# jacobkrantz/VLN-CE

Measured on AMD Instinct MI355X. Metric: policy-steps/sec (fwd+bwd), higher is better.
Workload: dtype f32

## Files before the change

### include/vlnce_hip.h

```cpp
#ifndef VLNCE_HIP_H
#define VLNCE_HIP_H

#include <stddef.h>
#include <stdint.h>

#ifdef __cplusplus
extern "C" {
#endif

typedef void* vlnce_stream_t;

enum { VLNCE_ACT_NONE = 0, VLNCE_ACT_RELU = 1, VLNCE_ACT_SIGMOID = 2, VLNCE_ACT_TANH = 3 };

int vlnce_version(void);
int vlnce_option_count(void);
int vlnce_option_index(const char* name);
const char* vlnce_last_error(void);

int vlnce_set_option(const char* name, int value);
int vlnce_get_option(const char* name, int* value);
int vlnce_option_default(const char* name, int* value);

typedef struct {
  int N, H, W, Cin;
  int Cout, KH, KW;
  int stride, pad;
  int Ho, Wo;
  int ldx, ldy;
} vlnce_conv_desc;

typedef struct {
  const float* x;
  int Cin, ldx;
  const void* w_frag;
  const float* in_scale;
  const float* in_shift;
  const float* in_center;
  int in_relu;
} vlnce_regen;

typedef struct {
  const float* in_scale;
  const float* in_shift;
  const float* in_center;
  int in_relu;
  const float* x2;
  const float* in2_scale;
  const float* in2_shift;
  const float* in2_center;
  float* side_out;
  const void* w_split;
  const void* w_frag;
  const int* options;
  int w_format;
  const vlnce_regen* regen;
} vlnce_prologue;

#define VLNCE_BN_SHARDS 16
typedef struct {
  double* acc;
  void* workspace;
  long workspace_bytes;
} vlnce_bn_sums;

typedef struct {
  const float* scale;
  const float* shift;
  const float* residual;
  int ldr;
  int act;
  int accumulate;
  float* stat_partial;
  const vlnce_bn_sums* bn;
  int stats_only;
} vlnce_epilogue;

long vlnce_conv2d_bn_workspace_bytes(const vlnce_conv_desc* d);
int vlnce_bn_finalize_sums(double* acc, int M, int C, const float* gamma, const float* beta,
                           float eps, float momentum, float* running_mean, float* running_var,
                           float* scale_out, float* shift_out, float* mean_out, float* rstd_out,
                           vlnce_stream_t stream);

int vlnce_conv2d_tiles_m(const vlnce_conv_desc* d);
int vlnce_conv2d_tile_rows(const vlnce_conv_desc* d);

int vlnce_conv2d_split_weights(const float* w, void* planes, long count, int format,
                               vlnce_stream_t stream);

long vlnce_conv2d_pack_bytes(const vlnce_conv_desc* d);
int vlnce_conv2d_pack_weights(const float* w_ohwi, void* frag, const vlnce_conv_desc* d,
                              int format , vlnce_stream_t stream);

typedef struct vlnce_weight_job {
  const float* w_oihw;
  void* dst;
  int Cout, Cin, T;
  int kind;
  int transposed;
  int format;
} vlnce_weight_job;
long vlnce_weight_job_items(const vlnce_weight_job* job);
int vlnce_conv2d_prepare_weights(const vlnce_weight_job* jobs_dev, const long* first_item_dev,
                                 int njobs, long total_items, vlnce_stream_t stream);

#define VLNCE_CONV_PATH_F32 0
#define VLNCE_CONV_PATH_X3 1
#define VLNCE_CONV_PATH_P3 2
#define VLNCE_CONV_PATH_M3 3
int vlnce_conv2d_last_path(void);

#define VLNCE_CONV_KERNEL(family, format, kernel, a, b, c) \
  ((family) | ((format) << 2) | ((kernel) << 4) | ((a) << 8) | ((b) << 16) | ((c) << 24))
#define VLNCE_CONV_KERNEL_FAMILY(v) ((v) & 3)
#define VLNCE_CONV_KERNEL_FORMAT(v) (((v) >> 2) & 3)
#define VLNCE_CONV_KERNEL_KIND(v) (((v) >> 4) & 15)
#define VLNCE_CONV_KERNEL_A(v) (((v) >> 8) & 255)
#define VLNCE_CONV_KERNEL_B(v) (((v) >> 16) & 255)
#define VLNCE_CONV_KERNEL_C(v) (((v) >> 24) & 127)
#define VLNCE_CONV_KERNEL_P3 0
#define VLNCE_CONV_KERNEL_U3 1
#define VLNCE_CONV_KERNEL_S3 2
#define VLNCE_CONV_KERNEL_R3 3
#define VLNCE_CONV_P3_DENSE 0
#define VLNCE_CONV_P3_GATHER 1
#define VLNCE_CONV_P3_DUAL 2
#define VLNCE_CONV_KERNEL_F32_BUF 0
#define VLNCE_CONV_KERNEL_F32_SPLITK 1
#define VLNCE_CONV_KERNEL_F32_V4 2
#define VLNCE_CONV_KERNEL_F32_S 3
#define VLNCE_CONV_KERNEL_F32_STEM3 4
#define VLNCE_CONV_KERNEL_F32_STEM1 5
#define VLNCE_CONV_KERNEL_F32_DUAL 6
int vlnce_conv2d_last_kernel(void);

int vlnce_conv2d_fwd(const float* x, const float* w_ohwi, float* y,
                     const vlnce_conv_desc* d, const vlnce_prologue* pro,
                     const vlnce_epilogue* epi, vlnce_stream_t stream);

int vlnce_gemm(const float* A, int lda, int transA, const float* B, int ldb, int transB,
               float* C, int ldc, int M, int N, int K,
               const vlnce_epilogue* epi, vlnce_stream_t stream);

#define VLNCE_GEMM_KERNEL(a, b, tile, splitk, zero, pass2) \
  ((a) | ((b) << 2) | ((tile) << 4) | ((zero) ? 1 << 6 : 0) | ((pass2) ? 1 << 7 : 0) | ((splitk) << 8))
#define VLNCE_GEMM_KERNEL_A(v) ((v) & 3)
#define VLNCE_GEMM_KERNEL_B(v) (((v) >> 2) & 3)
#define VLNCE_GEMM_KERNEL_TILE(v) (((v) >> 4) & 3)
#define VLNCE_GEMM_KERNEL_ZERO(v) (((v) >> 6) & 1)
#define VLNCE_GEMM_KERNEL_PASS2(v) (((v) >> 7) & 1)
#define VLNCE_GEMM_KERNEL_SPLITK(v) (((v) >> 8) & 255)
#define VLNCE_GEMM_A_BUF 0
#define VLNCE_GEMM_A_IM2COL_V4 1
#define VLNCE_GEMM_A_IM2COL_S 2
#define VLNCE_GEMM_A_TRANS 3
#define VLNCE_GEMM_B_BUF 0
#define VLNCE_GEMM_B_NK_V4 1
#define VLNCE_GEMM_B_NK_S 2
#define VLNCE_GEMM_B_KN 3
#define VLNCE_GEMM_TILE_128X128 1
#define VLNCE_GEMM_TILE_128X64 2
#define VLNCE_GEMM_TILE_64X64 3
int vlnce_gemm_last_kernel(void);

int vlnce_linear_rows_supported(int M, int N, int K);
int vlnce_linear_rows_fwd(const float* x, int ldx, const float* w, int ldw, const float* bias,
                          int act, float* y, int ldy, int M, int N, int K, vlnce_stream_t stream);
int vlnce_linear_rows_bwd(const float* x, int ldx, const float* w, int ldw, const float* dy,
                          int lddy, const float* y, int ldy, int act, float* dx, float* dw,
                          float* db, int M, int N, int K, vlnce_stream_t stream);

int vlnce_colsum(const float* x, int ldx, int M, int N, float* out, int accumulate,
                 vlnce_stream_t stream);

size_t vlnce_bn_finalize_workspace_bytes(int tiles_m, int C);
int vlnce_bn_finalize(const float* stat_partial, int tiles_m, int tile_rows, int M, int C,
                      const float* gamma, const float* beta, float eps, float momentum,
                      float* running_mean, float* running_var,
                      float* scale_out, float* shift_out,
                      float* mean_out, float* rstd_out,
                      void* workspace, size_t workspace_bytes,
                      vlnce_stream_t stream);

int vlnce_scale_shift_act(const float* x, const float* scale, const float* shift,
                          const float* center, int rows_per_sample, const float* residual,
                          float* y, long M, int C, int act, vlnce_stream_t stream);

int vlnce_scale_shift_add_act(const float* x1, const float* scale1, const float* shift1,
                              const float* center1, const float* x2, const float* scale2,
                              const float* shift2, const float* center2, float* y, long M, int C,
                              int act, vlnce_stream_t stream);

int vlnce_gn_chunks(int HW);
int vlnce_gn_partial(const float* x, int Nimg, int HW, int C, float* partial ,
                     vlnce_stream_t stream);
int vlnce_gn_finalize(const float* partial, int Nimg, int HW, int C, int groups,
                      const float* gamma, const float* beta, float eps,
                      float* scale_out, float* shift_out,
                      float* center_out,
                      float* mean_out, float* rstd_out,
                      vlnce_stream_t stream);
int vlnce_gn_finalize_tiles(const float* stat_partial, int tile_rows, int Nimg, int HW, int C,
                            int groups, const float* gamma, const float* beta, float eps,
                            float* scale_out, float* shift_out, float* center_out,
                            float* mean_out, float* rstd_out, vlnce_stream_t stream);
int vlnce_group_norm_small(const float* x, int Nimg, int HW, int C, int groups, const float* gamma,
                           const float* beta, float eps, const float* residual, int act, float* y,
                           vlnce_stream_t stream);

int vlnce_maxpool3x3s2(const float* x, float* y, int N, int H, int W, int C, int Ho, int Wo,
                       const float* in_scale, const float* in_shift, const float* in_center,
                       int in_relu, vlnce_stream_t stream);
int vlnce_avgpool2x2(const float* x, float* y, int N, int H, int W, int C, vlnce_stream_t stream);

int vlnce_space_to_depth2(const float* x, float* y, int N, int H, int W, int C, int pad_lo,
                          int pad_hi, const float* scale, const float* shift,
                          vlnce_stream_t stream);
#define VLNCE_DT_F32 0
#define VLNCE_DT_U8 1
typedef struct {
  const void* x;
  const void* x2;
  const unsigned char* mask2;
  int dtype;
  int N, F, Hs, Ws, C;
  int y0, x0, H, W;
} vlnce_frames;
int vlnce_frames_s2d(const vlnce_frames* frames, float* y, int pad_lo, int pad_hi,
                     const float* scale, const float* shift, vlnce_stream_t stream);
int vlnce_stem7_fwd(const vlnce_frames* frames, const float* in_scale, const float* in_shift,
                    const void* w_frag, int w_format, float* y, int Cout, const vlnce_epilogue* epi,
                    vlnce_stream_t stream);
int vlnce_frames_avgpool2(const vlnce_frames* frames, float* y, vlnce_stream_t stream);
int vlnce_frames_f32(const vlnce_frames* frames, float* y, const float* scale, const float* shift,
                     vlnce_stream_t stream);
int vlnce_frames_gather(const void* const* srcs, int F, int elem_bytes, int N, int Hs, int Ws,
                        int C, int y0, int x0, int H, int W, void* out, vlnce_stream_t stream);

int vlnce_frames_resize_area(const void* x, int dtype, int NF, int Hs, int Ws, int C, int OH, int OW,
                             int y0, int x0, int H, int W, void* out, vlnce_stream_t stream);

int vlnce_adaptive_avgpool(const float* x, float* y, int N, int H, int W, int C, int OH, int OW,
                           int ldy, vlnce_stream_t stream);

int vlnce_conv2d_wgrad(const float* x, const float* dy, float* dw_ohwi, const vlnce_conv_desc* d,
                       const float* dy_pow2, int P, int accumulate, vlnce_stream_t stream);
#define VLNCE_WGRAD_PATH_F32 0
#define VLNCE_WGRAD_PATH_X6_BF16 1
#define VLNCE_WGRAD_PATH_X6_F16 2
int vlnce_conv2d_wgrad_last_path(void);
#define VLNCE_WGRAD_KERNEL(path, tm, split) ((path) | ((tm) << 4) | ((split) ? 1 << 12 : 0))
#define VLNCE_WGRAD_KERNEL_PATH(v) ((v) & 15)
#define VLNCE_WGRAD_KERNEL_TM(v) (((v) >> 4) & 255)
#define VLNCE_WGRAD_KERNEL_SPLIT(v) (((v) >> 12) & 1)
int vlnce_conv2d_wgrad_last_kernel(void);
size_t vlnce_bn_bwd_workspace_floats(long M, int C);
int vlnce_bn_bwd(const float* dy, const float* y, const float* x, const float* mean,
                 const float* rstd, const float* gamma, long M, int C, int relu,
                 int use_batch_stats, float* dx, float* dres, float* dgamma, float* dbeta,
                 float* workspace, float* pow2, int P, vlnce_stream_t stream);
size_t vlnce_gn_bwd_workspace_floats(int Nimg, int HW, int C, int groups);
int vlnce_gn_bwd(const float* dy, const float* y, const float* x, const float* mean,
                 const float* rstd, const float* gamma, int Nimg, int HW, int C, int groups,
                 int relu, float* dx, float* dres, float* dgamma, float* dbeta, float* workspace,
                 float* pow2, int P, vlnce_stream_t stream);
int vlnce_maxpool3x3s2_argmax(const float* x, float* y, uint8_t* argmax, int N, int H, int W,
                              int C, int Ho, int Wo, vlnce_stream_t stream);
int vlnce_maxpool3x3s2_bwd(const float* dy, const uint8_t* argmax, float* dx, int N, int H, int W,
                           int C, int Ho, int Wo, vlnce_stream_t stream);
int vlnce_adaptive_avgpool_bwd(const float* dy, float* dx, int N, int H, int W, int C, int OH,
                               int OW, vlnce_stream_t stream);

int vlnce_action_head_fwd(const float* x, int ldx, const float* w, const float* b, int M, int K,
                          int A, float* logits_out, int* nan_count, vlnce_stream_t stream);
int vlnce_action_head_bwd(const float* x, int ldx, const float* w, const float* logits,
                          const float* dlogits, int M, int K, int A, float* dx, float* dw,
                          float* db, vlnce_stream_t stream);

int vlnce_attn_fwd(const float* q, const float* K, int ldk, const float* V, int ldv,
                   const uint8_t* mask, int mask_mode, float scale,
                   float* out, float* attn_out, int B, int P, int Dk, int Dv,
                   vlnce_stream_t stream);
int vlnce_attn_bwd(const float* dout, const float* q, const float* K, int ldk,
                   const float* V, int ldv, const uint8_t* mask, int mask_mode, float scale,
                   const float* attn, float* dq, float* dK, int lddk, float* dV, int lddv,
                   int B, int P, int Dk, int Dv, vlnce_stream_t stream);

int vlnce_attn_fwd_shared(const float* q, const float* K, int ldk, const float* V, int ldv,
                          const uint8_t* mask, int mask_mode, float scale, const int64_t* kv_index,
                          float* out, float* attn_out, int B, int P, int Dk, int Dv,
                          vlnce_stream_t stream);
int vlnce_attn_bwd_shared(const float* dout, const float* q, const float* K, int ldk,
                          const float* V, int ldv, const uint8_t* mask, int mask_mode, float scale,
                          const int64_t* kv_index, const float* attn, float* dq, float* dK,
                          int lddk, float* dV, int lddv, int B, int P, int Dk, int Dv,
                          vlnce_stream_t stream);
int vlnce_segment_sum(const float* x, const int64_t* index, int B, int U, long row_elems,
                      float* out, vlnce_stream_t stream);
int vlnce_rowzero_mask(const float* x, int ld, long rows, int C, uint8_t* mask,
                       vlnce_stream_t stream);

int vlnce_gru_gates_fwd(const float* gi, const float* gh, const float* h_prev,
                        const uint8_t* mask,
                        float* h_out, float* gates_out ,
                        float* hn_out ,
                        int B, int H, vlnce_stream_t stream);
int vlnce_gru_gates_bwd(const float* dh_out, const float* gates, const float* hn,
                        const float* h_prev, const uint8_t* mask,
                        float* dgi, float* dgh, float* dh_prev, int B, int H,
                        vlnce_stream_t stream);
int vlnce_lstm_gates_fwd(const float* gi, const float* gh, const float* c_prev,
                         const uint8_t* mask, float* h_out, float* c_out,
                         float* gates_out , int B, int H,
                         vlnce_stream_t stream);
int vlnce_lstm_gates_bwd(const float* dh_out, const float* dc_out, const float* gates,
                         const float* c_prev, const float* c_out, const uint8_t* mask,
                         float* dgates , float* dc_prev, int B, int H,
                         vlnce_stream_t stream);

int vlnce_rnn_seq_supported(int kind, int H);
int vlnce_rnn_seq_fwd(int kind, int dirs, const float* const* gi, const float* const* w_hh,
                      const float* const* b_hh, const int* lengths, float* const* out,
                      float* const* h_final, float* const* gates_save, float* const* aux_save,
                      int B, int L, int H, vlnce_stream_t stream);
int vlnce_rnn_seq_bwd(int kind, int dirs, const float* const* w_hh_t, const int* lengths,
                      const float* const* out, const float* const* gates_save,
                      const float* const* aux_save, const float* const* dout,
                      const float* const* dh_final, float* const* dgi, float* const* dgh,
                      int B, int L, int H, vlnce_stream_t stream);
int vlnce_rnn_seq_fwd2(int kind, int dirs, const float* const* gi, const float* const* w_hh,
                       const float* const* b_hh, const int* lengths, float* const* out_tm,
                       float* seq, long seq_st, long seq_sb, float* const* h_final,
                       float* const* gates_save, float* const* aux_save, int B, int L, int H,
                       vlnce_stream_t stream);
int vlnce_rnn_seq_bwd2(int kind, int dirs, const float* const* w_hh, const int* lengths,
                       const float* const* out_tm, const float* const* gates_save,
                       const float* const* aux_save, const float* dseq, long dseq_st, long dseq_sb,
                       float* dout_ws ,
                       const float* const* dh_final, float* const* dgi, float* const* dgh,
                       int B, int L, int H, vlnce_stream_t stream);
int vlnce_rnn_seq_wgrad(int kind, int dirs, int first_dir, const float* const* dgi, const float* const* dgh,
                        const float* const* out_tm, const float* x_tm, int ldx, int E,
                        const float* const* w_ih, float* const* dw_ih, float* const* dw_hh,
                        float* const* db_ih, float* const* db_hh, float* dx_tm, int B, int L, int H,
                        vlnce_stream_t stream);

int vlnce_mean_rows(const float* x, float* y, int B, int P, int C, vlnce_stream_t stream);
int vlnce_rnn_step_supported(int N, int H, int lstm);
int vlnce_rnn_step_fwd(int lstm, const float* gi, const float* h_prev, const float* c_prev,
                       const uint8_t* mask, const float* w_hh, const float* b_hh, float* hp_out,
                       float* h_out, float* aux_out, float* gates_out, int N, int H,
                       vlnce_stream_t stream);
int vlnce_rnn_step_bwd(int lstm, const float* dout, float* carry, const float* dc,
                       const float* gates, const float* aux, const float* hp, const float* c_prev,
                       const uint8_t* mask, const float* w_hh_t, float* dgi, float* dgh,
                       float* acc0, float* dc_prev, int N, int H, vlnce_stream_t stream);
int vlnce_mask_rows(const float* x, const uint8_t* mask, float* out, int B, int H,
                    vlnce_stream_t stream);
int vlnce_gru_rollout_supported(int N, int H);
long vlnce_gru_rollout_workspace_bytes(int N, int H);
int vlnce_gru_rollout_fwd(const float* gi, const float* h0, const uint8_t* mask, const float* w_hh,
                          const float* b_hh, float* hp, float* out, float* gates, float* aux,
                          void* workspace, int T, int N, int H, vlnce_stream_t stream);
int vlnce_gru_rollout_bwd(const float* dout, const float* dh_final, const float* gates,
                          const float* aux, const float* hp, const uint8_t* mask,
                          const float* w_hh_t, float* dgi, float* dgh, float* dh0,
                          void* workspace, int T, int N, int H, vlnce_stream_t stream);
int vlnce_lstm_rollout_supported(int N, int H);
long vlnce_lstm_rollout_workspace_bytes(int N, int H);
int vlnce_lstm_rollout_fwd(const float* gi, const float* h0, const float* c0, const uint8_t* mask,
                           const float* w_hh, const float* b_hh, float* hp, float* out, float* gates,
                           float* aux, void* workspace, int T, int N, int H, vlnce_stream_t stream);
int vlnce_lstm_rollout_bwd(const float* dout, const float* dh_final, const float* dc_final,
                           const float* gates, const float* aux, const float* hp, const float* c0,
                           const uint8_t* mask, const float* w_hh_t, float* dgi, float* dh0,
                           float* dc0, void* workspace, int T, int N, int H, vlnce_stream_t stream);

int vlnce_select_rows(const uint8_t* mask, const float* a, const float* b, float* out, int B, int H,
                      vlnce_stream_t stream);
int vlnce_embedding_bwd(const long* tokens, const float* grad_rows, float* grad_weight, long rows,
                        int E, long padding_idx, long vocab, vlnce_stream_t stream);
int vlnce_act_bwd(const float* dy, const float* y, float* dz, long n, int act,
                  vlnce_stream_t stream);

enum { VLNCE_SRC_F32 = 0, VLNCE_SRC_F16 = 1, VLNCE_SRC_I64 = 2 };
int vlnce_ragged_pad_rows(const void* src, int src_dtype, const int* offsets, int B, int Tmax,
                          long D, float fill, float* dst, vlnce_stream_t stream);
int vlnce_ragged_pad_rows_i64(const int64_t* src, const int* offsets, int B, int Tmax, long D,
                              int64_t fill, int64_t* dst, vlnce_stream_t stream);
int vlnce_dagger_targets(const int64_t* oracle_actions, const int* offsets, int B, int Tmax,
                         float inflection_coef, int64_t* corrected_out, float* weights_out,
                         uint8_t* masks_out, vlnce_stream_t stream);

enum { VLNCE_TRAJ_F32 = 0, VLNCE_TRAJ_F16 = 1, VLNCE_TRAJ_I64 = 2, VLNCE_TRAJ_U8 = 3 };
#define VLNCE_TRAJ_MAX_SENSORS 8
#define VLNCE_TRAJ_MAX_ROWS 128
typedef struct {
  const void* src;
  void* dst;
  long row_stride, c_stride, p_stride;
  int C, P;
  int src_dtype;
  int dst_dtype;
} vlnce_traj_sensor;
int vlnce_traj_append(const vlnce_traj_sensor* sensors, int n_sensors, const int* slots,
                      const int* steps, int n_rows, long capacity, vlnce_stream_t stream);
int vlnce_dagger_mix_actions(const int64_t* actions, const void* expert, int expert_dtype,
                             const float* uniform, float beta, int n, int64_t* prev_actions,
                             int64_t* stepped , vlnce_stream_t stream);

int vlnce_ppo_returns(const float* rewards, float* value_preds, const float* masks,
                      const float* next_value, float* returns, int T, int N, float gamma, float tau,
                      int use_gae, vlnce_stream_t stream);

int vlnce_ppo_loss(const float* values, const float* returns, const float* value_preds,
                   const float* logp, const float* old_logp, const float* adv,
                   const float* ent_pano, const float* ent_offset, const float* ent_distance,
                   const float* radians, int B, float clip, float value_coef, float entropy_coef,
                   float pano_coef, float offset_coef, float distance_coef, float reg_coef,
                   int use_clipped, float* stats, float* grads, vlnce_stream_t stream);

int vlnce_il_loss_supported(int T, int N, int A);
int vlnce_il_loss(const float* logits, const int64_t* targets, const float* weights,
                  const float* aux, float inv_scalar, int T, int N, int A, float* stats,
                  float* dlogits, vlnce_stream_t stream);

int vlnce_pair_mse(const float* estimate, const float* target, const uint8_t* mask, int E, int R,
                   float* value, float* d_estimate, vlnce_stream_t stream);

#ifdef __cplusplus
}
#endif
#endif
```

### vln-ce_amd/_lib.py

```python
import collections
import ctypes as C
import os
import threading

import torch

_HERE = os.path.dirname(os.path.abspath(__file__))
LIB_PATH = os.environ.get("VLNCE_HIP_LIB") or os.path.join(_HERE, "libvlnce_hip.so")

_P = C.c_void_p
_I = C.c_int
_F = C.c_float
_L = C.c_long


def _buffer_format(explicit, *bufs):
    tags = {getattr(b, "_vlnce_fmt", None) for b in bufs if b is not None} - {None}
    if explicit:
        tags.add(int(explicit))
    if len(tags) > 1:
        raise RuntimeError(f"weight buffers / w_format disagree on the plane format: {sorted(tags)}")
    return tags.pop() if tags else 1


ConvKernel = collections.namedtuple("ConvKernel", "family kernel fmt a b c")
ConvKernel.__doc__ = """family: "f32" | "x3" | "p3" | "m3" (= conv2d_last_path()); kernel: the kernel within it
("conv_p3" | "conv_u3" | "conv_s3", "conv_m3", "conv_x3", "buf" | "splitk" | "v4" | "s" | "stem3" |
"stem1" | "dual" of igemm_kernel); fmt: plane format 1 / 2 (0: fp32); a, b, c per kernel:
  conv_p3: tile 1..6, mode "dense" | "gather" | "dual", 0      conv_u3: rows, kind 0..2, waves
  conv_s3: Cin, 1 = statistics only, 0      conv_r3: regenerated Cin, Cout / 32, skip kind 1 / 2
  conv_m3: NT, KSPLIT, RB      conv_x3: tile 1..4, dual 0 / 1, 0
  splitk: the split factor, 0, 0"""
WgradKernel = collections.namedtuple("WgradKernel", "path tm split")

_FAMILIES = ("f32", "x3", "p3", "m3")
_KERNELS = {"f32": ("buf", "splitk", "v4", "s", "stem3", "stem1", "dual"), "x3": ("conv_x3",),
            "p3": ("conv_p3", "conv_u3", "conv_s3", "conv_r3"), "m3": ("conv_m3",)}
_P3_MODES = ("dense", "gather", "dual")


def decode_conv_kernel(v):
    if v < 0:
        return None
    family = _FAMILIES[v & 3]
    kernel = _KERNELS[family][(v >> 4) & 15]
    a, b, c = (v >> 8) & 255, (v >> 16) & 255, (v >> 24) & 127
    if kernel == "conv_p3":
        b = _P3_MODES[b]
    return ConvKernel(family, kernel, (v >> 2) & 3, a, b, c)


def decode_wgrad_kernel(v):
    return None if v < 0 else WgradKernel(v & 15, (v >> 4) & 255, bool((v >> 12) & 1))


GemmKernel = collections.namedtuple("GemmKernel", "a b tile splitk zero pass2")
GemmKernel.__doc__ = """a: the A loader "buf" | "v4" | "s" | "trans"; b: the B loader "buf" | "nk_v4" | "nk_s" | "kn";
tile: (rows, columns) of the igemm_kernel instance; splitk: the split-K factor (1 = not split); zero: C was
zero-filled first; pass2: the second bias / activation pass ran"""
_GEMM_A = ("buf", "v4", "s", "trans")
_GEMM_B = ("buf", "nk_v4", "nk_s", "kn")
_GEMM_TILES = (None, (128, 128), (128, 64), (64, 64))


def decode_gemm_kernel(v):
    if v < 0:
        return None
    return GemmKernel(_GEMM_A[v & 3], _GEMM_B[(v >> 2) & 3], _GEMM_TILES[(v >> 4) & 3], (v >> 8) & 255,
                      bool((v >> 6) & 1), bool((v >> 7) & 1))


class ConvDesc(C.Structure):
    _fields_ = [(n, _I) for n in
                ("N", "H", "W", "Cin", "Cout", "KH", "KW", "stride", "pad", "Ho", "Wo", "ldx", "ldy")]


class WeightJob(C.Structure):
    _fields_ = [("w_oihw", _P), ("dst", _P), ("Cout", _I), ("Cin", _I), ("T", _I), ("kind", _I),
                ("transposed", _I), ("format", _I)]


class WeightPrepPlan:
    __slots__ = ("table", "first_item", "njobs", "total", "keep")


class Prologue(C.Structure):
    _fields_ = [("in_scale", _P), ("in_shift", _P), ("in_center", _P), ("in_relu", _I),
                ("x2", _P), ("in2_scale", _P), ("in2_shift", _P), ("in2_center", _P),
                ("side_out", _P), ("w_split", _P), ("w_frag", _P), ("options", _P), ("w_format", _I),
                ("regen", _P)]


class Regen(C.Structure):
    _fields_ = [("x", _P), ("Cin", _I), ("ldx", _I), ("w_frag", _P), ("in_scale", _P), ("in_shift", _P),
                ("in_center", _P), ("in_relu", _I)]


class Frames(C.Structure):
    _fields_ = [("x", _P), ("x2", _P), ("mask2", _P), ("dtype", _I), ("N", _I), ("F", _I),
                ("Hs", _I), ("Ws", _I), ("C", _I), ("y0", _I), ("x0", _I), ("H", _I), ("W", _I)]


class BnSums(C.Structure):
    _fields_ = [("acc", _P), ("workspace", _P), ("workspace_bytes", _L)]


class TrajSensor(C.Structure):
    _fields_ = [("src", _P), ("dst", _P), ("row_stride", _L), ("c_stride", _L), ("p_stride", _L),
                ("C", _I), ("P", _I), ("src_dtype", _I), ("dst_dtype", _I)]


class Epilogue(C.Structure):
    _fields_ = [("scale", _P), ("shift", _P), ("residual", _P), ("ldr", _I), ("act", _I),
                ("accumulate", _I), ("stat_partial", _P), ("bn", C.POINTER(BnSums)),
                ("stats_only", _I)]


_SIGNATURES = {
    "vlnce_version": (_I, []),
    "vlnce_last_error": (C.c_char_p, []),
    "vlnce_set_option": (_I, [C.c_char_p, _I]),
    "vlnce_get_option": (_I, [C.c_char_p, C.POINTER(_I)]),
    "vlnce_option_default": (_I, [C.c_char_p, C.POINTER(_I)]),
    "vlnce_conv2d_split_weights": (_I, [_P, _P, C.c_long, _I, _P]),
    "vlnce_conv2d_last_path": (_I, []),
    "vlnce_conv2d_wgrad_last_path": (_I, []),
    "vlnce_conv2d_last_kernel": (_I, []),
    "vlnce_conv2d_wgrad_last_kernel": (_I, []),
    "vlnce_gemm_last_kernel": (_I, []),
    "vlnce_embedding_bwd": (_I, [_P, _P, _P, _L, _I, _L, _L, _P]),
    "vlnce_conv2d_pack_bytes": (C.c_long, [C.POINTER(ConvDesc)]),
    "vlnce_conv2d_pack_weights": (_I, [_P, _P, C.POINTER(ConvDesc), _I, _P]),
    "vlnce_weight_job_items": (C.c_long, [C.POINTER(WeightJob)]),
    "vlnce_conv2d_prepare_weights": (_I, [_P, _P, _I, C.c_long, _P]),
    "vlnce_conv2d_tiles_m": (_I, [C.POINTER(ConvDesc)]),
    "vlnce_conv2d_tile_rows": (_I, [C.POINTER(ConvDesc)]),
    "vlnce_conv2d_bn_workspace_bytes": (C.c_long, [C.POINTER(ConvDesc)]),
    "vlnce_bn_finalize_sums": (_I, [_P, _I, _I, _P, _P, _F, _F, _P, _P, _P, _P, _P, _P, _P]),
    "vlnce_conv2d_fwd": (_I, [_P, _P, _P, C.POINTER(ConvDesc), C.POINTER(Prologue),
                              C.POINTER(Epilogue), _P]),
    "vlnce_gemm": (_I, [_P, _I, _I, _P, _I, _I, _P, _I, _I, _I, _I, C.POINTER(Epilogue), _P]),
    "vlnce_colsum": (_I, [_P, _I, _I, _I, _P, _I, _P]),
    "vlnce_bn_finalize_workspace_bytes": (C.c_size_t, [_I, _I]),
    "vlnce_bn_finalize": (_I, [_P, _I, _I, _I, _I, _P, _P, _F, _F, _P, _P, _P, _P, _P, _P, _P,
                               C.c_size_t, _P]),
    "vlnce_scale_shift_act": (_I, [_P, _P, _P, _P, _I, _P, _P, _L, _I, _I, _P]),
    "vlnce_gn_chunks": (_I, [_I]),
    "vlnce_gn_partial": (_I, [_P, _I, _I, _I, _P, _P]),
    "vlnce_gn_finalize": (_I, [_P, _I, _I, _I, _I, _P, _P, _F, _P, _P, _P, _P, _P, _P]),
    "vlnce_gn_finalize_tiles": (_I, [_P, _I, _I, _I, _I, _I, _P, _P, _F, _P, _P, _P, _P, _P, _P]),
    "vlnce_maxpool3x3s2": (_I, [_P, _P, _I, _I, _I, _I, _I, _I, _P, _P, _P, _I, _P]),
    "vlnce_scale_shift_add_act": (_I, [_P, _P, _P, _P, _P, _P, _P, _P, _P, _L, _I, _I, _P]),
    "vlnce_avgpool2x2": (_I, [_P, _P, _I, _I, _I, _I, _P]),
    "vlnce_ragged_pad_rows": (_I, [_P, _I, _P, _I, _I, _L, _F, _P, _P]),
    "vlnce_ragged_pad_rows_i64": (_I, [_P, _P, _I, _I, _L, _L, _P, _P]),
    "vlnce_dagger_targets": (_I, [_P, _P, _I, _I, _F, _P, _P, _P, _P]),
    "vlnce_traj_append": (_I, [C.POINTER(TrajSensor), _I, C.POINTER(_I), C.POINTER(_I), _I, _L, _P]),
    "vlnce_dagger_mix_actions": (_I, [_P, _P, _I, _P, _F, _I, _P, _P, _P]),
    "vlnce_ppo_loss": (_I, [_P, _P, _P, _P, _P, _P, _P, _P, _P, _P, _I, _F, _F, _F, _F, _F, _F, _F, _I,
                            _P, _P, _P]),
    "vlnce_ppo_returns": (_I, [_P, _P, _P, _P, _P, _I, _I, _F, _F, _I, _P]),
    "vlnce_il_loss_supported": (_I, [_I, _I, _I]),
    "vlnce_il_loss": (_I, [_P, _P, _P, _P, _F, _I, _I, _I, _P, _P, _P]),
    "vlnce_pair_mse": (_I, [_P, _P, _P, _I, _I, _P, _P, _P]),
    "vlnce_space_to_depth2": (_I, [_P, _P, _I, _I, _I, _I, _I, _I, _P, _P, _P]),
    "vlnce_frames_s2d": (_I, [C.POINTER(Frames), _P, _I, _I, _P, _P, _P]),
    "vlnce_frames_avgpool2": (_I, [C.POINTER(Frames), _P, _P]),
    "vlnce_stem7_fwd": (_I, [C.POINTER(Frames), _P, _P, _P, _I, _P, _I, C.POINTER(Epilogue), _P]),
    "vlnce_frames_f32": (_I, [C.POINTER(Frames), _P, _P, _P, _P]),
    "vlnce_frames_gather": (_I, [_P, _I, _I, _I, _I, _I, _I, _I, _I, _I, _I, _P, _P]),
    "vlnce_frames_resize_area": (_I, [_P] + [_I] * 11 + [_P, _P]),
    "vlnce_adaptive_avgpool": (_I, [_P, _P, _I, _I, _I, _I, _I, _I, _I, _P]),
    "vlnce_attn_fwd": (_I, [_P, _P, _I, _P, _I, _P, _I, _F, _P, _P, _I, _I, _I, _I, _P]),
    "vlnce_attn_bwd": (_I, [_P, _P, _P, _I, _P, _I, _P, _I, _F, _P, _P, _P, _I, _P, _I,
                            _I, _I, _I, _I, _P]),
    "vlnce_rowzero_mask": (_I, [_P, _I, _L, _I, _P, _P]),
    "vlnce_attn_fwd_shared": (_I, [_P, _P, _I, _P, _I, _P, _I, _F, _P, _P, _P, _I, _I, _I, _I, _P]),
    "vlnce_attn_bwd_shared": (_I, [_P, _P, _P, _I, _P, _I, _P, _I, _F, _P, _P, _P, _P, _I, _P, _I,
                                   _I, _I, _I, _I, _P]),
    "vlnce_segment_sum": (_I, [_P, _P, _I, _I, _L, _P, _P]),
    "vlnce_action_head_fwd": (_I, [_P, _I, _P, _P, _I, _I, _I, _P, _P, _P]),
    "vlnce_action_head_bwd": (_I, [_P, _I, _P, _P, _P, _I, _I, _I, _P, _P, _P, _P]),
    "vlnce_gru_gates_fwd": (_I, [_P, _P, _P, _P, _P, _P, _P, _I, _I, _P]),
    "vlnce_gru_gates_bwd": (_I, [_P, _P, _P, _P, _P, _P, _P, _P, _I, _I, _P]),
    "vlnce_lstm_gates_fwd": (_I, [_P, _P, _P, _P, _P, _P, _P, _I, _I, _P]),
    "vlnce_lstm_gates_bwd": (_I, [_P, _P, _P, _P, _P, _P, _P, _P, _I, _I, _P]),
    "vlnce_mean_rows": (_I, [_P, _P, _I, _I, _I, _P]),
    "vlnce_mask_rows": (_I, [_P, _P, _P, _I, _I, _P]),
    "vlnce_conv2d_wgrad": (_I, [_P, _P, _P, C.POINTER(ConvDesc), _P, _I, _I, _P]),
    "vlnce_bn_bwd": (_I, [_P, _P, _P, _P, _P, _P, _L, _I, _I, _I, _P, _P, _P, _P, _P, _P, _I, _P]),
    "vlnce_bn_bwd_workspace_floats": (C.c_size_t, [_L, _I]),
    "vlnce_gn_bwd_workspace_floats": (C.c_size_t, [_I, _I, _I, _I]),
    "vlnce_gn_bwd": (_I, [_P, _P, _P, _P, _P, _P, _I, _I, _I, _I, _I, _P, _P, _P, _P, _P, _P, _I, _P]),
    "vlnce_maxpool3x3s2_argmax": (_I, [_P, _P, _P, _I, _I, _I, _I, _I, _I, _P]),
    "vlnce_maxpool3x3s2_bwd": (_I, [_P, _P, _P, _I, _I, _I, _I, _I, _I, _P]),
    "vlnce_adaptive_avgpool_bwd": (_I, [_P, _P, _I, _I, _I, _I, _I, _I, _P]),
    "vlnce_rnn_seq_supported": (_I, [_I, _I]),
    "vlnce_rnn_seq_fwd": (_I, [_I, _I, _P, _P, _P, _P, _P, _P, _P, _P, _I, _I, _I, _P]),
    "vlnce_rnn_seq_bwd": (_I, [_I, _I, _P, _P, _P, _P, _P, _P, _P, _P, _P, _I, _I, _I, _P]),
    "vlnce_option_count": (_I, []),
    "vlnce_option_index": (_I, [C.c_char_p]),
    "vlnce_linear_rows_supported": (_I, [_I, _I, _I]),
    "vlnce_linear_rows_fwd": (_I, [_P, _I, _P, _I, _P, _I, _P, _I, _I, _I, _I, _P]),
    "vlnce_linear_rows_bwd": (_I, [_P, _I, _P, _I, _P, _I, _P, _I, _I, _P, _P, _P, _I, _I, _I, _P]),
    "vlnce_rnn_seq_fwd2": (_I, [_I, _I, _P, _P, _P, _P, _P, _P, _L, _L, _P, _P, _P, _I, _I, _I, _P]),
    "vlnce_rnn_seq_bwd2": (_I, [_I, _I, _P, _P, _P, _P, _P, _P, _L, _L, _P, _P, _P, _P, _I, _I, _I, _P]),
    "vlnce_rnn_seq_wgrad": (_I, [_I, _I, _I, _P, _P, _P, _P, _I, _I, _P, _P, _P, _P, _P, _P, _I, _I, _I, _P]),
    "vlnce_group_norm_small": (_I, [_P, _I, _I, _I, _I, _P, _P, _F, _P, _I, _P, _P]),
    "vlnce_gru_rollout_supported": (_I, [_I, _I]),
    "vlnce_gru_rollout_workspace_bytes": (C.c_long, [_I, _I]),
    "vlnce_gru_rollout_fwd": (_I, [_P, _P, _P, _P, _P, _P, _P, _P, _P, _P, _I, _I, _I, _P]),
    "vlnce_gru_rollout_bwd": (_I, [_P, _P, _P, _P, _P, _P, _P, _P, _P, _P, _P, _I, _I, _I, _P]),
    "vlnce_lstm_rollout_supported": (_I, [_I, _I]),
    "vlnce_lstm_rollout_workspace_bytes": (C.c_long, [_I, _I]),
    "vlnce_lstm_rollout_fwd": (_I, [_P, _P, _P, _P, _P, _P, _P, _P, _P, _P, _P, _I, _I, _I, _P]),
    "vlnce_lstm_rollout_bwd": (_I, [_P, _P, _P, _P, _P, _P, _P, _P, _P, _P, _P, _P, _P, _I, _I, _I, _P]),
    "vlnce_rnn_step_supported": (_I, [_I, _I, _I]),
    "vlnce_rnn_step_fwd": (_I, [_I, _P, _P, _P, _P, _P, _P, _P, _P, _P, _P, _I, _I, _P]),
    "vlnce_rnn_step_bwd": (_I, [_I, _P, _P, _P, _P, _P, _P, _P, _P, _P, _P, _P, _P, _P, _I, _I, _P]),
    "vlnce_select_rows": (_I, [_P, _P, _P, _P, _I, _I, _P]),
    "vlnce_act_bwd": (_I, [_P, _P, _P, _L, _I, _P]),
}


def collapse_rows(t):
    while True:
        groups = []
        for n, st in zip(t.shape[1:], t.stride()[1:]):
            if n == 1:
                continue
            if groups and groups[-1][1] == st * n:
                groups[-1] = (groups[-1][0] * n, int(st))
            else:
                groups.append((int(n), int(st)))
        if len(groups) <= 2:
            break
        t = t.contiguous()
    row_stride = int(t.stride(0)) if t.size(0) > 1 else 0
    if not groups:
        return t, row_stride, 1, 0, 1, 0
    if len(groups) == 1:
        return t, row_stride, groups[0][0], groups[0][1], 1, 0
    return t, row_stride, groups[0][0], groups[0][1], groups[1][0], groups[1][1]


def exported_symbols():
    return sorted(_SIGNATURES)


def load_cdll(path=LIB_PATH):
    if not os.path.exists(path):
        raise RuntimeError(
            f"{path} not found: build it with `python __graft_entry__.py` (hipcc, gfx950). "
            "The VLN-CE policy path has no CPU fallback."
        )
    dll = C.CDLL(path)
    for name, (res, args) in _SIGNATURES.items():
        fn = getattr(dll, name)
        fn.restype = res
        fn.argtypes = args
    return dll


class _CallState(threading.local):
    dev = None
    restore = None


_CALL = _CallState()


def _ptr(t):
    if t is None:
        return None
    if not t.is_cuda:
        raise RuntimeError("libvlnce_hip: tensor is not on a GPU (no CPU fallback)")
    idx = t.device.index
    if _CALL.dev is None:
        _CALL.dev = idx
    elif _CALL.dev != idx:
        first, _CALL.dev = _CALL.dev, None
        raise RuntimeError(f"libvlnce_hip: tensors of one call live on cuda:{first} and "
                           f"cuda:{idx}")
    return t.data_ptr()


def _stream():
    dev, _CALL.dev = _CALL.dev, None
    if dev is None:
        return torch.cuda.current_stream().cuda_stream
    cur = torch.cuda.current_device()
    if dev != cur:
        _CALL.restore = cur
        torch.cuda.set_device(dev)
    return torch.cuda.current_stream(dev).cuda_stream


def _leave_device():
    if _CALL.restore is not None:
        cur, _CALL.restore = _CALL.restore, None
        torch.cuda.set_device(cur)


class HipLib:

    name = "hip"

    ABI = 150

    def __init__(self, path=LIB_PATH):
        self.dll = load_cdll(path)
        have = int(self.dll.vlnce_version())
        if have != self.ABI:
            raise RuntimeError(f"{path} has ABI {have}, this package binds ABI {self.ABI}: "
                               "rebuild it (python __graft_entry__.py)")

        self._conv_math = None
        self._tls = threading.local()
        self._options_from_env()

    OPTION_NAMES = ("conv_math", "p3", "p3_tile", "s3", "u3", "u3_waves", "x3_tile", "igemm_tile",
                    "igemm_nobuf", "igemm_no_splitk", "wgrad_tile", "rollout_one_xcd", "m3", "r3",
                    "s3_wgs")

    def _options_from_env(self):
        for name in self.OPTION_NAMES:
            v = os.environ.get("VLNCE_" + name.upper())
            if v is None:
                continue
            if name == "conv_math":
                v = {"f32": 0, "0": 0, "bf16": 1, "1": 1, "f16": 2, "2": 2}.get(v.strip().lower(), v)
            elif name in ("igemm_nobuf", "igemm_no_splitk"):
                v = 0 if v in ("", "0") else 1
            try:
                v = int(v)
            except ValueError:
                import warnings
                warnings.warn(f"VLNCE_{name.upper()}={v!r} is not an integer: ignored "
                              f"(the option keeps its default)")
                continue
            self.set_option(name, v)

    def set_option(self, name, value):
        self._check(self.dll.vlnce_set_option(name.encode(), int(value)), "vlnce_set_option")
        if name == "conv_math":
            self._conv_math = int(value)

    def plane_format(self, options=None):
        v = None
        if options:
            v = options.get("conv_math")
        if v is None:
            sc = getattr(self._tls, "scoped", None)
            if sc:
                v = sc.get("conv_math")
        if v is None or v < 0:
            v = self._conv_math
            if v is None:
                v = self._conv_math = self.get_option("conv_math")
        return 2 if v == 2 else 1

    def effective_option(self, name):
        sc = getattr(self._tls, "scoped", None)
        if sc and sc.get(name, -1) >= 0:
            return int(sc[name])
        return self.get_option(name)

    def get_option(self, name):
        v = _I(0)
        self._check(self.dll.vlnce_get_option(name.encode(), C.byref(v)), "vlnce_get_option")
        return v.value

    def option_default(self, name):
        v = _I(0)
        self._check(self.dll.vlnce_option_default(name.encode(), C.byref(v)), "vlnce_option_default")
        return v.value

    PER_LAUNCH = ("conv_math", "p3", "p3_tile", "s3", "u3", "u3_waves", "x3_tile", "m3", "r3", "s3_wgs")

    def _launch_options(self, overrides):
        if not overrides:
            return None
        arr = (C.c_int * int(self.dll.vlnce_option_count()))(*([-1] * int(self.dll.vlnce_option_count())))
        for name, v in overrides.items():
            i = int(self.dll.vlnce_option_index(name.encode()))
            if i < 0:
                raise RuntimeError(f"unknown dispatch option {name!r}")
            arr[i] = int(v)
        return arr

    def options(self, **kw):
        lib = self
        unknown = [k for k in kw if k not in self.OPTION_NAMES]
        if unknown:
            raise RuntimeError(f"unknown dispatch option(s) {unknown}")

        class _Scope:
            def __enter__(self_inner):
                self_inner.prev = getattr(lib._tls, "scoped", None)
                scoped = dict(self_inner.prev or {})
                scoped.update({k: v for k, v in kw.items() if k in lib.PER_LAUNCH})
                lib._tls.scoped = scoped or None
                self_inner.old = {k: lib.get_option(k) for k in kw if k not in lib.PER_LAUNCH}
                for k in self_inner.old:
                    lib.set_option(k, kw[k])
                return lib

            def __exit__(self_inner, *exc):
                lib._tls.scoped = self_inner.prev
                for k, v in self_inner.old.items():
                    lib.set_option(k, v)
                return False

        return _Scope()

    def _check(self, rc, what):
        _leave_device()
        if rc != 0:
            raise RuntimeError(f"{what} failed (rc={rc}): {self.dll.vlnce_last_error().decode()}")

    @staticmethod
    def _desc(g):
        return ConvDesc(*[int(g[k]) for k, _ in ConvDesc._fields_])

    def conv2d_tiles(self, g):
        d = self._desc(g)
        return self.dll.vlnce_conv2d_tiles_m(C.byref(d)), self.dll.vlnce_conv2d_tile_rows(C.byref(d))

    def conv2d_fwd(self, x, w, y, g, in_scale=None, in_shift=None, in_relu=0, scale=None,
                   shift=None, residual=None, ldr=0, act=0, accumulate=0, stat_partial=None,
                   in_center=None, x2=None, in2_scale=None, in2_shift=None, in2_center=None,
                   side_out=None, w_split=None, w_frag=None, bn=None, options=None, w_format=None,
                   stats_only=False, regen=None):
        d = self._desc(g)
        w_format = _buffer_format(w_format, w_split, w_frag, regen["w_frag"] if regen else None)
        rg = None
        if regen is not None:
            rx = regen["x"]
            rg = Regen(_ptr(rx), rx.size(-1), rx.size(-1), _ptr(regen["w_frag"]),
                       _ptr(regen.get("in_scale")), _ptr(regen.get("in_shift")),
                       _ptr(regen.get("in_center")), int(regen.get("in_relu", 0)))
        opts = self._launch_options(options if options is not None
                                    else getattr(self._tls, "scoped", None))
        pro = Prologue(_ptr(in_scale), _ptr(in_shift), _ptr(in_center), int(in_relu), _ptr(x2),
                       _ptr(in2_scale), _ptr(in2_shift), _ptr(in2_center), _ptr(side_out),
                       _ptr(w_split), _ptr(w_frag),
                       C.cast(opts, C.c_void_p) if opts is not None else None, int(w_format),
                       C.cast(C.pointer(rg), C.c_void_p) if rg is not None else None)
        bnp = None
        if bn is not None:
            acc, ws = bn
            bnp = C.pointer(BnSums(_ptr(acc), _ptr(ws), ws.numel() * ws.element_size()))
        epi = Epilogue(_ptr(scale), _ptr(shift), _ptr(residual), int(ldr), int(act),
                       int(accumulate), _ptr(stat_partial), bnp, int(bool(stats_only)))
        self._check(self.dll.vlnce_conv2d_fwd(_ptr(x), _ptr(w), _ptr(y), C.byref(d), C.byref(pro),
                                              C.byref(epi), _stream()), "vlnce_conv2d_fwd")

    def bn_finalize_sums(self, acc, M, gamma, beta, eps, momentum, running_mean, running_var,
                         scale_out, mean_out, shift_out=None, rstd_out=None):
        Cc = scale_out.numel()
        self._check(self.dll.vlnce_bn_finalize_sums(
            _ptr(acc), int(M), Cc, _ptr(gamma), _ptr(beta), float(eps), float(momentum),
            _ptr(running_mean), _ptr(running_var), _ptr(scale_out), _ptr(shift_out),
            _ptr(mean_out), _ptr(rstd_out), _stream()), "vlnce_bn_finalize_sums")

    def conv2d_bn_workspace_bytes(self, g):
        d = self._desc(g)
        return int(self.dll.vlnce_conv2d_bn_workspace_bytes(C.byref(d)))

    def conv2d_split_weights(self, w, planes, fmt=1):
        self._check(self.dll.vlnce_conv2d_split_weights(_ptr(w), _ptr(planes), w.numel(), int(fmt),
                                                        _stream()), "vlnce_conv2d_split_weights")

    def conv2d_last_path(self):
        return int(self.dll.vlnce_conv2d_last_path())

    def conv2d_wgrad_last_path(self):
        return int(self.dll.vlnce_conv2d_wgrad_last_path())

    def conv2d_last_kernel(self):
        return decode_conv_kernel(int(self.dll.vlnce_conv2d_last_kernel()))

    def conv2d_wgrad_last_kernel(self):
        return decode_wgrad_kernel(int(self.dll.vlnce_conv2d_wgrad_last_kernel()))

    def conv2d_pack_bytes(self, g):
        d = self._desc(g)
        return int(self.dll.vlnce_conv2d_pack_bytes(C.byref(d)))

    def conv2d_pack_weights(self, w, frag, g, fmt=1):
        d = self._desc(g)
        self._check(self.dll.vlnce_conv2d_pack_weights(_ptr(w), _ptr(frag), C.byref(d), int(fmt),
                                                       _stream()), "vlnce_conv2d_pack_weights")

    WP_F32, WP_PLANES, WP_FRAGMENTS = 0, 1, 2

    def weight_prep_plan(self, jobs):
        arr = (WeightJob * len(jobs))()
        first = [0]
        for j, (w, dst, kind, transposed, fmt) in zip(arr, jobs):
            assert w.is_cuda and w.is_contiguous() and w.dtype == torch.float32 and w.dim() == 4
            j.w_oihw, j.dst = w.data_ptr(), dst.data_ptr()
            j.Cout, j.Cin, j.T = w.size(0), w.size(1), w.size(2) * w.size(3)
            j.kind, j.transposed, j.format = int(kind), int(bool(transposed)), int(fmt or 0)
            items = int(self.dll.vlnce_weight_job_items(C.byref(j)))
            if items <= 0:
                raise ValueError(f"weight_prep_plan: job not eligible: {tuple(w.shape)} kind={kind} "
                                 f"transposed={transposed} format={fmt}")
            first.append(first[-1] + items)
        plan = WeightPrepPlan()
        dev = jobs[0][1].device
        plan.table = torch.frombuffer(bytearray(bytes(arr)), dtype=torch.uint8).to(dev)
        plan.first_item = torch.tensor(first, dtype=torch.int64).to(dev)
        plan.njobs, plan.total = len(jobs), first[-1]
        plan.keep = [(w, dst) for w, dst, *_ in jobs]
        return plan

    def conv2d_prepare_weights(self, plan):
        self._check(self.dll.vlnce_conv2d_prepare_weights(_ptr(plan.table), _ptr(plan.first_item),
                                                          plan.njobs, plan.total, _stream()),
                    "vlnce_conv2d_prepare_weights")

    def gemm(self, A, lda, transA, B, ldb, transB, Cm, ldc, M, N, K, scale=None, shift=None,
             residual=None, ldr=0, act=0, accumulate=0):
        epi = Epilogue(_ptr(scale), _ptr(shift), _ptr(residual), int(ldr), int(act),
                       int(accumulate), None)
        self._check(self.dll.vlnce_gemm(_ptr(A), lda, transA, _ptr(B), ldb, transB, _ptr(Cm), ldc,
                                        M, N, K, C.byref(epi), _stream()), "vlnce_gemm")

    def gemm_last_kernel(self):
        return decode_gemm_kernel(int(self.dll.vlnce_gemm_last_kernel()))

    def colsum(self, x, ldx, M, N, out, accumulate=0):
        self._check(self.dll.vlnce_colsum(_ptr(x), ldx, M, N, _ptr(out), accumulate, _stream()),
                    "vlnce_colsum")

    def bn_finalize_workspace_bytes(self, tiles_m, Cc):
        return int(self.dll.vlnce_bn_finalize_workspace_bytes(tiles_m, Cc))

    def bn_finalize(self, partial, tiles_m, tile_rows, M, Cc, gamma, beta, eps, momentum,
                    running_mean, running_var, scale_out, shift_out, mean_out=None, rstd_out=None,
                    workspace=None):
        wb = workspace.numel() * workspace.element_size() if workspace is not None else 0
        self._check(self.dll.vlnce_bn_finalize(
            _ptr(partial), tiles_m, tile_rows, M, Cc, _ptr(gamma), _ptr(beta), eps, momentum,
            _ptr(running_mean), _ptr(running_var), _ptr(scale_out), _ptr(shift_out),
            _ptr(mean_out), _ptr(rstd_out), _ptr(workspace), wb, _stream()), "vlnce_bn_finalize")

    def scale_shift_act(self, x, scale, shift, rows_per_sample, residual, y, M, Cc, act,
                        center=None):
        self._check(self.dll.vlnce_scale_shift_act(
            _ptr(x), _ptr(scale), _ptr(shift), _ptr(center), rows_per_sample, _ptr(residual),
            _ptr(y), M, Cc, act, _stream()), "vlnce_scale_shift_act")

    def gn_chunks(self, HW):
        return self.dll.vlnce_gn_chunks(HW)

    def gn_partial(self, x, Nimg, HW, Cc, partial):
        self._check(self.dll.vlnce_gn_partial(_ptr(x), Nimg, HW, Cc, _ptr(partial), _stream()),
                    "vlnce_gn_partial")

    def gn_finalize(self, partial, Nimg, HW, Cc, groups, gamma, beta, eps, scale_out, shift_out,
                    mean_out=None, rstd_out=None, center_out=None):
        self._check(self.dll.vlnce_gn_finalize(
            _ptr(partial), Nimg, HW, Cc, groups, _ptr(gamma), _ptr(beta), eps, _ptr(scale_out),
            _ptr(shift_out), _ptr(center_out), _ptr(mean_out), _ptr(rstd_out), _stream()),
            "vlnce_gn_finalize")

    def gn_finalize_tiles(self, partial, tile_rows, Nimg, HW, Cc, groups, gamma, beta, eps,
                          scale_out, shift_out, mean_out=None, rstd_out=None, center_out=None):
        self._check(self.dll.vlnce_gn_finalize_tiles(
            _ptr(partial), tile_rows, Nimg, HW, Cc, groups, _ptr(gamma), _ptr(beta), eps,
            _ptr(scale_out), _ptr(shift_out), _ptr(center_out), _ptr(mean_out), _ptr(rstd_out),
            _stream()), "vlnce_gn_finalize_tiles")

    def maxpool3x3s2(self, x, y, N, H, W, Cc, Ho, Wo, in_scale=None, in_shift=None, in_relu=0,
                     in_center=None):
        self._check(self.dll.vlnce_maxpool3x3s2(_ptr(x), _ptr(y), N, H, W, Cc, Ho, Wo,
                                                _ptr(in_scale), _ptr(in_shift), _ptr(in_center),
                                                int(in_relu), _stream()), "vlnce_maxpool3x3s2")

    def scale_shift_add_act(self, x1, s1, t1, x2, s2, t2, y, M, Cc, act, c1=None, c2=None):
        self._check(self.dll.vlnce_scale_shift_add_act(
            _ptr(x1), _ptr(s1), _ptr(t1), _ptr(c1), _ptr(x2), _ptr(s2), _ptr(t2), _ptr(c2),
            _ptr(y), M, Cc, act, _stream()), "vlnce_scale_shift_add_act")

    _SRC = {torch.float32: 0, torch.float16: 1, torch.int64: 2}

    def ragged_pad_rows(self, src, offsets, B, Tmax, D, fill, dst):
        assert offsets.dtype == torch.int32 and dst.dtype == torch.float32
        self._check(self.dll.vlnce_ragged_pad_rows(
            _ptr(src), self._SRC[src.dtype], _ptr(offsets), B, Tmax, D, float(fill),
            _ptr(dst), _stream()), "vlnce_ragged_pad_rows")

    def ragged_pad_rows_i64(self, src, offsets, B, Tmax, D, fill, dst):
        assert src.dtype == torch.int64 and dst.dtype == torch.int64
        self._check(self.dll.vlnce_ragged_pad_rows_i64(
            _ptr(src), _ptr(offsets), B, Tmax, D, int(fill), _ptr(dst), _stream()),
            "vlnce_ragged_pad_rows_i64")

    def dagger_targets(self, oracle, offsets, B, Tmax, coef, corrected, weights, masks):
        self._check(self.dll.vlnce_dagger_targets(
            _ptr(oracle), _ptr(offsets), B, Tmax, float(coef), _ptr(corrected),
            _ptr(weights), _ptr(masks), _stream()), "vlnce_dagger_targets")

    _TRAJ = {torch.float32: 0, torch.float16: 1, torch.int64: 2, torch.uint8: 3}
    TRAJ_MAX_SENSORS, TRAJ_MAX_ROWS = 8, 128

    def traj_append(self, sources, arenas, slots, steps):
        n = len(slots)
        assert len(sources) == len(arenas) and len(steps) == n and n > 0
        capacity, num_envs = int(arenas[0].size(1)), min(int(a.size(0)) for a in arenas)
        if min(slots) < 0 or max(slots) >= num_envs:
            raise RuntimeError(f"traj_append: slot outside the arena's {num_envs} environments")
        table, keep = [], []
        for src, dst in zip(sources, arenas):
            src, rs, Cc, cs, P, ps = collapse_rows(src)
            keep.append(src)
            if src.size(0) != n:
                raise RuntimeError(f"traj_append: {src.size(0)} source rows for {n} slots")
            if dst.dim() != 3 or not dst.is_contiguous() or dst.size(1) != capacity \
                    or dst.size(2) != Cc * P:
                raise RuntimeError(f"traj_append: arena {tuple(dst.shape)} for rows of {Cc * P} "
                                   f"elements at capacity {capacity}")
            if src.dtype not in (torch.float32, torch.int64, torch.uint8) \
                    or dst.dtype not in (torch.float16, torch.float32, torch.int64):
                raise RuntimeError(f"traj_append: {src.dtype} -> {dst.dtype} is not a recorded pair")
            table.append((src, dst, rs, Cc, cs, P, ps))
        for r0 in range(0, n, self.TRAJ_MAX_ROWS):
            r1 = min(n, r0 + self.TRAJ_MAX_ROWS)
            sl = (_I * (r1 - r0))(*[int(v) for v in slots[r0:r1]])
            stp = (_I * (r1 - r0))(*[int(v) for v in steps[r0:r1]])
            for k0 in range(0, len(table), self.TRAJ_MAX_SENSORS):
                part = table[k0:k0 + self.TRAJ_MAX_SENSORS]
                arr = (TrajSensor * len(part))()
                for a, (src, dst, rs, Cc, cs, P, ps) in zip(arr, part):
                    a.src = _ptr(src) + r0 * rs * src.element_size()
                    a.dst = _ptr(dst)
                    a.row_stride, a.c_stride, a.p_stride, a.C, a.P = rs, cs, ps, Cc, P
                    a.src_dtype, a.dst_dtype = self._TRAJ[src.dtype], self._TRAJ[dst.dtype]
                self._check(self.dll.vlnce_traj_append(arr, len(part), sl, stp, r1 - r0, capacity,
                                                       _stream()), "vlnce_traj_append")

    def dagger_mix_actions(self, actions, expert, uniform, beta, prev_actions, stepped):
        n = actions.numel()
        assert actions.dtype == torch.int64 and prev_actions.dtype == torch.int64
        assert stepped.dtype == torch.int64 and stepped.numel() == 2 * n and stepped.is_contiguous()
        assert uniform.dtype == torch.float32 and expert.dtype in (torch.float32, torch.int64)
        assert expert.numel() == n and uniform.numel() == n and prev_actions.numel() == n
        assert all(t.is_contiguous() for t in (actions, expert, uniform, prev_actions))
        self._check(self.dll.vlnce_dagger_mix_actions(
            _ptr(actions), _ptr(expert), self._TRAJ[expert.dtype], _ptr(uniform), float(beta), n,
            _ptr(prev_actions), _ptr(stepped), _stream()), "vlnce_dagger_mix_actions")

    def ppo_loss(self, values, returns, value_preds, logp, old_logp, adv, ent_pano, ent_offset,
                 ent_distance, radians, B, clip, value_coef, entropy_coef, pano_coef, offset_coef,
                 distance_coef, reg_coef, use_clipped, stats, grads):
        self._check(self.dll.vlnce_ppo_loss(
            _ptr(values), _ptr(returns), _ptr(value_preds), _ptr(logp), _ptr(old_logp), _ptr(adv),
            _ptr(ent_pano), _ptr(ent_offset), _ptr(ent_distance), _ptr(radians), B, clip, value_coef,
            entropy_coef, pano_coef, offset_coef, distance_coef, reg_coef, int(use_clipped),
            _ptr(stats), _ptr(grads), _stream()), "vlnce_ppo_loss")

    def ppo_returns(self, rewards, value_preds, masks, next_value, returns, T, N, gamma, tau,
                    use_gae):
        self._check(self.dll.vlnce_ppo_returns(_ptr(rewards), _ptr(value_preds), _ptr(masks),
                                               _ptr(next_value), _ptr(returns), T, N, float(gamma),
                                               float(tau), int(use_gae), _stream()),
                    "vlnce_ppo_returns")

    def il_loss_supported(self, T, N, A):
        return bool(self.dll.vlnce_il_loss_supported(int(T), int(N), int(A)))

    def il_loss(self, logits, targets, weights, aux, inv_scalar, T, N, A, stats, dlogits):
        assert logits.dtype == torch.float32 and weights.dtype == torch.float32
        assert targets.dtype == torch.int64 and (aux is None or aux.dtype == torch.float32)
        assert logits.numel() == T * N * A and targets.numel() == T * N and weights.numel() == T * N
        assert stats.numel() == 3 and dlogits.numel() == T * N * A
        assert all(t.is_contiguous() for t in (logits, targets, weights, stats, dlogits))
        self._check(self.dll.vlnce_il_loss(_ptr(logits), _ptr(targets), _ptr(weights), _ptr(aux),
                                           float(inv_scalar), T, N, A, _ptr(stats), _ptr(dlogits),
                                           _stream()), "vlnce_il_loss")

    def pair_mse(self, estimate, target, mask, E, R, value, d_estimate):
        assert estimate.dtype == torch.float32 and target.dtype == torch.float32
        assert mask.dtype in (torch.bool, torch.uint8) and mask.numel() == E
        assert estimate.numel() == E and target.numel() == R and d_estimate.numel() == E
        assert all(t.is_contiguous() for t in (estimate, target, mask, d_estimate))
        self._check(self.dll.vlnce_pair_mse(_ptr(estimate), _ptr(target), _ptr(mask), E, R,
                                            _ptr(value), _ptr(d_estimate), _stream()),
                    "vlnce_pair_mse")

    def space_to_depth2(self, x, y, N, H, W, Cc, pad_lo, pad_hi, scale=None, shift=None):
        self._check(self.dll.vlnce_space_to_depth2(_ptr(x), _ptr(y), N, H, W, Cc, pad_lo, pad_hi,
                                                   _ptr(scale), _ptr(shift), _stream()),
                    "vlnce_space_to_depth2")

    _DT = {torch.float32: 0, torch.uint8: 1}

    def _frames(self, fr):
        x = fr["x"]
        if fr.get("x2") is not None and fr["x2"].dtype != x.dtype:
            raise RuntimeError("libvlnce_hip: frames and the extra frame differ in dtype")
        return Frames(_ptr(x), _ptr(fr.get("x2")), _ptr(fr.get("mask2")), self._DT[x.dtype],
                      *[int(fr[k]) for k in ("N", "F", "Hs", "Ws", "C", "y0", "x0", "H", "W")])

    def frames_s2d(self, fr, y, pad_lo, pad_hi, scale=None, shift=None):
        d = self._frames(fr)
        self._check(self.dll.vlnce_frames_s2d(C.byref(d), _ptr(y), pad_lo, pad_hi, _ptr(scale),
                                              _ptr(shift), _stream()), "vlnce_frames_s2d")

    def stem7_fwd(self, fr, in_scale, in_shift, w_frag, y, scale=None, shift=None, act=0, bn=None,
                  w_format=None):
        d = self._frames(fr)
        w_format = _buffer_format(w_format, w_frag)
        bnp = None
        if bn is not None:
            bnp = C.pointer(BnSums(_ptr(bn), None, 0))
        epi = Epilogue(_ptr(scale), _ptr(shift), None, 0, int(act), 0, None, bnp)
        self._check(self.dll.vlnce_stem7_fwd(C.byref(d), _ptr(in_scale), _ptr(in_shift),
                                             _ptr(w_frag), int(w_format), _ptr(y), y.size(-1),
                                             C.byref(epi), _stream()), "vlnce_stem7_fwd")

    def frames_avgpool2(self, fr, y):
        d = self._frames(fr)
        self._check(self.dll.vlnce_frames_avgpool2(C.byref(d), _ptr(y), _stream()),
                    "vlnce_frames_avgpool2")

    def frames_f32(self, fr, y, scale=None, shift=None):
        d = self._frames(fr)
        self._check(self.dll.vlnce_frames_f32(C.byref(d), _ptr(y), _ptr(scale), _ptr(shift),
                                              _stream()), "vlnce_frames_f32")

    def frames_gather(self, srcs, elem_bytes, N, Hs, Ws, Cc, y0, x0, H, W, out):
        arr = (C.c_void_p * len(srcs))(*[_ptr(t) for t in srcs])
        self._check(self.dll.vlnce_frames_gather(arr, len(srcs), elem_bytes, N, Hs, Ws, Cc, y0, x0,
                                                 H, W, _ptr(out), _stream()), "vlnce_frames_gather")

    def frames_resize_area(self, x, is_u8, NF, Hs, Ws, Cc, OH, OW, y0, x0, H, W, out):
        self._check(self.dll.vlnce_frames_resize_area(_ptr(x), 1 if is_u8 else 0, NF, Hs, Ws, Cc, OH,
                                                      OW, y0, x0, H, W, _ptr(out), _stream()),
                    "vlnce_frames_resize_area")

    def avgpool2x2(self, x, y, N, H, W, Cc):
        self._check(self.dll.vlnce_avgpool2x2(_ptr(x), _ptr(y), N, H, W, Cc, _stream()),
                    "vlnce_avgpool2x2")

    def adaptive_avgpool(self, x, y, N, H, W, Cc, OH, OW, ldy):
        self._check(self.dll.vlnce_adaptive_avgpool(_ptr(x), _ptr(y), N, H, W, Cc, OH, OW, ldy,
                                                    _stream()), "vlnce_adaptive_avgpool")

    def mean_rows(self, x, y, B, P, Cc):
        self._check(self.dll.vlnce_mean_rows(_ptr(x), _ptr(y), B, P, Cc, _stream()),
                    "vlnce_mean_rows")

    def action_head_fwd(self, x, ldx, w, b, M, K, A, logits_out, nan_count=None):
        self._check(self.dll.vlnce_action_head_fwd(_ptr(x), ldx, _ptr(w), _ptr(b), M, K, A,
                                                   _ptr(logits_out), _ptr(nan_count), _stream()),
                    "vlnce_action_head_fwd")

    def action_head_bwd(self, x, ldx, w, logits, dlogits, M, K, A, dx=None, dw=None, db=None):
        self._check(self.dll.vlnce_action_head_bwd(_ptr(x), ldx, _ptr(w), _ptr(logits),
                                                   _ptr(dlogits), M, K, A, _ptr(dx), _ptr(dw),
                                                   _ptr(db), _stream()), "vlnce_action_head_bwd")

    def attn_fwd(self, q, K, ldk, V, ldv, mask, mask_mode, scale, out, attn_out, B, P, Dk, Dv,
                 kv_index=None):
        if kv_index is not None:
            self._check(self.dll.vlnce_attn_fwd_shared(
                _ptr(q), _ptr(K), ldk, _ptr(V), ldv, _ptr(mask), mask_mode, scale, _ptr(kv_index),
                _ptr(out), _ptr(attn_out), B, P, Dk, Dv, _stream()), "vlnce_attn_fwd_shared")
            return
        self._check(self.dll.vlnce_attn_fwd(_ptr(q), _ptr(K), ldk, _ptr(V), ldv, _ptr(mask),
                                            mask_mode, scale, _ptr(out), _ptr(attn_out), B, P, Dk,
                                            Dv, _stream()), "vlnce_attn_fwd")

    def segment_sum(self, x, index, B, U, row_elems, out):
        self._check(self.dll.vlnce_segment_sum(_ptr(x), _ptr(index), B, U, row_elems, _ptr(out),
                                               _stream()), "vlnce_segment_sum")

    def attn_bwd(self, dout, q, K, ldk, V, ldv, mask, mask_mode, scale, attn, dq, dK, lddk, dV,
                 lddv, B, P, Dk, Dv, kv_index=None):
        if kv_index is not None:
            self._check(self.dll.vlnce_attn_bwd_shared(
                _ptr(dout), _ptr(q), _ptr(K), ldk, _ptr(V), ldv, _ptr(mask), mask_mode, scale,
                _ptr(kv_index), _ptr(attn), _ptr(dq), _ptr(dK), lddk, _ptr(dV), lddv, B, P, Dk, Dv,
                _stream()), "vlnce_attn_bwd_shared")
            return
        self._check(self.dll.vlnce_attn_bwd(_ptr(dout), _ptr(q), _ptr(K), ldk, _ptr(V), ldv,
                                            _ptr(mask), mask_mode, scale, _ptr(attn), _ptr(dq),
                                            _ptr(dK), lddk, _ptr(dV), lddv, B, P, Dk, Dv,
                                            _stream()), "vlnce_attn_bwd")

    def rowzero_mask(self, x, ld, rows, Cc, mask):
        self._check(self.dll.vlnce_rowzero_mask(_ptr(x), ld, rows, Cc, _ptr(mask), _stream()),
                    "vlnce_rowzero_mask")

    def gru_gates_fwd(self, gi, gh, h_prev, mask, h_out, gates_out, hn_out, B, H):
        self._check(self.dll.vlnce_gru_gates_fwd(_ptr(gi), _ptr(gh), _ptr(h_prev), _ptr(mask),
                                                 _ptr(h_out), _ptr(gates_out), _ptr(hn_out), B, H,
                                                 _stream()), "vlnce_gru_gates_fwd")

    def gru_gates_bwd(self, dh_out, gates, hn, h_prev, mask, dgi, dgh, dh_prev, B, H):
        self._check(self.dll.vlnce_gru_gates_bwd(_ptr(dh_out), _ptr(gates), _ptr(hn), _ptr(h_prev),
                                                 _ptr(mask), _ptr(dgi), _ptr(dgh), _ptr(dh_prev),
                                                 B, H, _stream()), "vlnce_gru_gates_bwd")

    def lstm_gates_fwd(self, gi, gh, c_prev, mask, h_out, c_out, gates_out, B, H):
        self._check(self.dll.vlnce_lstm_gates_fwd(_ptr(gi), _ptr(gh), _ptr(c_prev), _ptr(mask),
                                                  _ptr(h_out), _ptr(c_out), _ptr(gates_out), B, H,
                                                  _stream()), "vlnce_lstm_gates_fwd")

    def lstm_gates_bwd(self, dh_out, dc_out, gates, c_prev, c_out, mask, dgates, dc_prev, B, H):
        self._check(self.dll.vlnce_lstm_gates_bwd(_ptr(dh_out), _ptr(dc_out), _ptr(gates),
                                                  _ptr(c_prev), _ptr(c_out), _ptr(mask),
                                                  _ptr(dgates), _ptr(dc_prev), B, H, _stream()),
                    "vlnce_lstm_gates_bwd")

    def mask_rows(self, x, mask, out, B, H):
        self._check(self.dll.vlnce_mask_rows(_ptr(x), _ptr(mask), _ptr(out), B, H, _stream()),
                    "vlnce_mask_rows")

    def conv2d_wgrad(self, x, dy, dw, g, dy_pow2=None, accumulate=False):
        d = self._desc(g)
        self._check(self.dll.vlnce_conv2d_wgrad(_ptr(x), _ptr(dy), _ptr(dw), C.byref(d),
                                                _ptr(dy_pow2),
                                                dy_pow2.size(1) if dy_pow2 is not None else 0,
                                                int(bool(accumulate)), _stream()),
                    "vlnce_conv2d_wgrad")

    def bn_bwd_workspace_floats(self, M, Cc):
        return int(self.dll.vlnce_bn_bwd_workspace_floats(M, Cc))

    def bn_bwd(self, dy, y, x, mean, rstd, gamma, M, Cc, relu, use_batch_stats, dx, dres, dgamma,
               dbeta, workspace=None, pow2=None):
        self._check(self.dll.vlnce_bn_bwd(_ptr(dy), _ptr(y), _ptr(x), _ptr(mean), _ptr(rstd),
                                          _ptr(gamma), M, Cc, int(relu), int(use_batch_stats),
                                          _ptr(dx), _ptr(dres), _ptr(dgamma), _ptr(dbeta),
                                          _ptr(workspace), _ptr(pow2),
                                          pow2.size(1) if pow2 is not None else 0, _stream()),
                    "vlnce_bn_bwd")

    def gn_bwd_workspace_floats(self, Nimg, HW, Cc, groups):
        return int(self.dll.vlnce_gn_bwd_workspace_floats(Nimg, HW, Cc, groups))

    def gn_bwd(self, dy, y, x, mean, rstd, gamma, Nimg, HW, Cc, groups, relu, dx, dres, dgamma,
               dbeta, workspace, pow2=None):
        self._check(self.dll.vlnce_gn_bwd(_ptr(dy), _ptr(y), _ptr(x), _ptr(mean), _ptr(rstd),
                                          _ptr(gamma), Nimg, HW, Cc, groups, int(relu), _ptr(dx),
                                          _ptr(dres), _ptr(dgamma), _ptr(dbeta), _ptr(workspace),
                                          _ptr(pow2), pow2.size(1) if pow2 is not None else 0,
                                          _stream()), "vlnce_gn_bwd")

    def maxpool3x3s2_argmax(self, x, y, argmax, N, H, W, Cc, Ho, Wo):
        self._check(self.dll.vlnce_maxpool3x3s2_argmax(_ptr(x), _ptr(y), _ptr(argmax), N, H, W, Cc,
                                                       Ho, Wo, _stream()),
                    "vlnce_maxpool3x3s2_argmax")

    def maxpool3x3s2_bwd(self, dy, argmax, dx, N, H, W, Cc, Ho, Wo):
        self._check(self.dll.vlnce_maxpool3x3s2_bwd(_ptr(dy), _ptr(argmax), _ptr(dx), N, H, W, Cc,
                                                    Ho, Wo, _stream()), "vlnce_maxpool3x3s2_bwd")

    def adaptive_avgpool_bwd(self, dy, dx, N, H, W, Cc, OH, OW):
        self._check(self.dll.vlnce_adaptive_avgpool_bwd(_ptr(dy), _ptr(dx), N, H, W, Cc, OH, OW,
                                                        _stream()), "vlnce_adaptive_avgpool_bwd")

    @staticmethod
    def _parr(ts, n):
        if ts is None:
            return None
        arr = (C.c_void_p * 2)()
        for i in range(n):
            arr[i] = _ptr(ts[i])
        return arr

    def rnn_seq_supported(self, kind, H):
        return bool(self.dll.vlnce_rnn_seq_supported(kind, H))

    def rnn_seq_fwd(self, kind, dirs, gi, w_hh, b_hh, lengths, out, h_final, gates_save, aux_save,
                    B, Lm, H):
        pa = self._parr
        self._check(self.dll.vlnce_rnn_seq_fwd(
            kind, dirs, pa(gi, dirs), pa(w_hh, dirs), pa(b_hh, dirs), _ptr(lengths), pa(out, dirs),
            pa(h_final, dirs), pa(gates_save, dirs), pa(aux_save, dirs), B, Lm, H, _stream()),
            "vlnce_rnn_seq_fwd")

    def rnn_seq_bwd(self, kind, dirs, w_hh_t, lengths, out, gates_save, aux_save, dout, dh_final,
                    dgi, dgh, B, Lm, H):
        pa = self._parr
        self._check(self.dll.vlnce_rnn_seq_bwd(
            kind, dirs, pa(w_hh_t, dirs), _ptr(lengths), pa(out, dirs), pa(gates_save, dirs),
            pa(aux_save, dirs), pa(dout, dirs), pa(dh_final, dirs), pa(dgi, dirs), pa(dgh, dirs),
            B, Lm, H, _stream()), "vlnce_rnn_seq_bwd")

    def linear_rows_supported(self, M, N, K):
        return bool(self.dll.vlnce_linear_rows_supported(M, N, K))

    def linear_rows_fwd(self, x, ldx, w, ldw, bias, act, y, ldy, M, N, K):
        self._check(self.dll.vlnce_linear_rows_fwd(_ptr(x), ldx, _ptr(w), ldw, _ptr(bias), act, _ptr(y),
                                                   ldy, M, N, K, _stream()), "vlnce_linear_rows_fwd")

    def linear_rows_bwd(self, x, ldx, w, ldw, dy, lddy, y, ldy, act, dx, dw, db, M, N, K):
        self._check(self.dll.vlnce_linear_rows_bwd(_ptr(x), ldx, _ptr(w), ldw, _ptr(dy), lddy, _ptr(y),
                                                   ldy, act, _ptr(dx), _ptr(dw), _ptr(db), M, N, K,
                                                   _stream()), "vlnce_linear_rows_bwd")

    def rnn_seq_fwd2(self, kind, dirs, gi, w_hh, b_hh, lengths, out_tm, seq, seq_st, seq_sb, h_final,
                     gates_save, aux_save, B, Lm, H):
        pa = self._parr
        self._check(self.dll.vlnce_rnn_seq_fwd2(
            kind, dirs, pa(gi, dirs), pa(w_hh, dirs), pa(b_hh, dirs), _ptr(lengths), pa(out_tm, dirs),
            _ptr(seq), seq_st, seq_sb, pa(h_final, dirs), pa(gates_save, dirs), pa(aux_save, dirs),
            B, Lm, H, _stream()), "vlnce_rnn_seq_fwd2")

    def rnn_seq_bwd2(self, kind, dirs, w_hh, lengths, out_tm, gates_save, aux_save, dseq, dseq_st,
                     dseq_sb, dout_ws, dh_final, dgi, dgh, B, Lm, H):
        pa = self._parr
        self._check(self.dll.vlnce_rnn_seq_bwd2(
            kind, dirs, pa(w_hh, dirs), _ptr(lengths), pa(out_tm, dirs), pa(gates_save, dirs),
            pa(aux_save, dirs), _ptr(dseq), dseq_st, dseq_sb, _ptr(dout_ws), pa(dh_final, dirs),
            pa(dgi, dirs), pa(dgh, dirs), B, Lm, H, _stream()), "vlnce_rnn_seq_bwd2")

    def rnn_seq_wgrad(self, kind, dirs, dgi, dgh, out_tm, x_tm, ldx, E, w_ih, dw_ih, dw_hh, db_ih,
                      db_hh, dx_tm, B, Lm, H, first_dir=0):
        pa = self._parr
        self._check(self.dll.vlnce_rnn_seq_wgrad(
            kind, dirs, first_dir, pa(dgi, dirs), pa(dgh, dirs), pa(out_tm, dirs), _ptr(x_tm), ldx, E,
            pa(w_ih, dirs), pa(dw_ih, dirs), pa(dw_hh, dirs), pa(db_ih, dirs), pa(db_hh, dirs),
            _ptr(dx_tm), B, Lm, H, _stream()), "vlnce_rnn_seq_wgrad")

    def group_norm_small(self, x, N, HW, Cc, groups, gamma, beta, eps, residual, act, y):
        self._check(self.dll.vlnce_group_norm_small(
            _ptr(x), N, HW, Cc, groups, _ptr(gamma), _ptr(beta), eps, _ptr(residual), act, _ptr(y),
            _stream()), "vlnce_group_norm_small")

    def gru_rollout_supported(self, N, H):
        if os.environ.get("VLNCE_GRU_ROLLOUT", "1") == "0":
            return False
        return bool(self.dll.vlnce_gru_rollout_supported(N, H))

    def gru_rollout_workspace_bytes(self, N, H):
        return int(self.dll.vlnce_gru_rollout_workspace_bytes(N, H))

    def gru_rollout_fwd(self, gi, h0, mask, w_hh, b_hh, hp, out, gates, aux, workspace, T, N, H):
        self._check(self.dll.vlnce_gru_rollout_fwd(
            _ptr(gi), _ptr(h0), _ptr(mask), _ptr(w_hh), _ptr(b_hh), _ptr(hp), _ptr(out),
            _ptr(gates), _ptr(aux), _ptr(workspace), T, N, H, _stream()), "vlnce_gru_rollout_fwd")

    def gru_rollout_bwd(self, dout, dh_final, gates, aux, hp, mask, w_hh_t, dgi, dgh, dh0,
                        workspace, T, N, H):
        self._check(self.dll.vlnce_gru_rollout_bwd(
            _ptr(dout), _ptr(dh_final), _ptr(gates), _ptr(aux), _ptr(hp), _ptr(mask),
            _ptr(w_hh_t), _ptr(dgi), _ptr(dgh), _ptr(dh0), _ptr(workspace), T, N, H, _stream()),
            "vlnce_gru_rollout_bwd")

    def lstm_rollout_supported(self, N, H):
        return bool(self.dll.vlnce_lstm_rollout_supported(N, H))

    def lstm_rollout_workspace_bytes(self, N, H):
        return int(self.dll.vlnce_lstm_rollout_workspace_bytes(N, H))

    def lstm_rollout_fwd(self, gi, h0, c0, mask, w_hh, b_hh, hp, out, gates, aux, workspace,
                         T, N, H):
        self._check(self.dll.vlnce_lstm_rollout_fwd(
            _ptr(gi), _ptr(h0), _ptr(c0), _ptr(mask), _ptr(w_hh), _ptr(b_hh), _ptr(hp), _ptr(out),
            _ptr(gates), _ptr(aux), _ptr(workspace), T, N, H, _stream()), "vlnce_lstm_rollout_fwd")

    def lstm_rollout_bwd(self, dout, dh_final, dc_final, gates, aux, hp, c0, mask, w_hh_t, dgi,
                         dh0, dc0, workspace, T, N, H):
        self._check(self.dll.vlnce_lstm_rollout_bwd(
            _ptr(dout), _ptr(dh_final), _ptr(dc_final), _ptr(gates), _ptr(aux), _ptr(hp), _ptr(c0),
            _ptr(mask), _ptr(w_hh_t), _ptr(dgi), _ptr(dh0), _ptr(dc0), _ptr(workspace), T, N, H,
            _stream()), "vlnce_lstm_rollout_bwd")

    def rnn_step_supported(self, N, H, lstm):
        if os.environ.get("VLNCE_RNN_STEP_FUSED", "1") == "0":
            return False
        return bool(self.dll.vlnce_rnn_step_supported(N, H, int(lstm)))

    def rnn_step_fwd(self, lstm, gi, h_prev, c_prev, mask, w_hh, b_hh, hp_out, h_out, aux_out,
                     gates_out, N, H):
        self._check(self.dll.vlnce_rnn_step_fwd(
            int(lstm), _ptr(gi), _ptr(h_prev), _ptr(c_prev), _ptr(mask), _ptr(w_hh), _ptr(b_hh),
            _ptr(hp_out), _ptr(h_out), _ptr(aux_out), _ptr(gates_out), N, H, _stream()),
            "vlnce_rnn_step_fwd")

    def rnn_step_bwd(self, lstm, dout, carry, dc, gates, aux, hp, c_prev, mask, w_hh_t, dgi, dgh,
                     acc0, dc_prev, N, H):
        self._check(self.dll.vlnce_rnn_step_bwd(
            int(lstm), _ptr(dout), _ptr(carry), _ptr(dc), _ptr(gates), _ptr(aux), _ptr(hp),
            _ptr(c_prev), _ptr(mask), _ptr(w_hh_t), _ptr(dgi), _ptr(dgh), _ptr(acc0),
            _ptr(dc_prev), N, H, _stream()), "vlnce_rnn_step_bwd")

    def select_rows(self, mask, a, b, out, B, H):
        self._check(self.dll.vlnce_select_rows(_ptr(mask), _ptr(a), _ptr(b), _ptr(out), B, H,
                                               _stream()), "vlnce_select_rows")

    def embedding_bwd(self, tokens, grad_rows, grad_weight, padding_idx):
        self._check(self.dll.vlnce_embedding_bwd(_ptr(tokens), _ptr(grad_rows), _ptr(grad_weight),
                                                 tokens.numel(), grad_weight.size(1),
                                                 -1 if padding_idx is None else int(padding_idx),
                                                 grad_weight.size(0), _stream()),
                    "vlnce_embedding_bwd")

    def act_bwd(self, dy, y, dz, n, act):
        self._check(self.dll.vlnce_act_bwd(_ptr(dy), _ptr(y), _ptr(dz), n, act, _stream()),
                    "vlnce_act_bwd")


_LIB = None


def get_lib():
    global _LIB
    if _LIB is None:
        _LIB = HipLib()
    return _LIB
```

### vln-ce_amd/csrc/api.cpp

```cpp
#include <stdarg.h>
#include <stdio.h>
#include <string.h>

#include <atomic>

#include "common_opts.h"

static thread_local char g_err[512] = "";

void vlnce_set_error(const char* fmt, ...) {
  va_list ap;
  va_start(ap, fmt);
  vsnprintf(g_err, sizeof(g_err), fmt, ap);
  va_end(ap);
}

extern "C" const char* vlnce_last_error(void) { return g_err; }
extern "C" int vlnce_version(void) { return 150; }

namespace {
struct OptDef {
  const char* name;
  int def;
};
const OptDef kOpts[VLNCE_OPT_COUNT] = {
    {"conv_math", 2},   {"p3", 2},          {"p3_tile", 0},         {"s3", 1},
    {"u3", 1},          {"u3_waves", 8},    {"x3_tile", 0},         {"igemm_tile", 0},
    {"igemm_nobuf", 0}, {"igemm_no_splitk", 0}, {"wgrad_tile", 64}, {"rollout_one_xcd", 0},
    {"m3", 1},          {"r3", 1},          {"s3_wgs", 0},
};
std::atomic<int> g_opt[VLNCE_OPT_COUNT] = {
    {2}, {2}, {0}, {1}, {1}, {8}, {0}, {0}, {0}, {0}, {64}, {0}, {1}, {1}, {0},
};
int opt_index(const char* name) {
  if (name)
    for (int i = 0; i < VLNCE_OPT_COUNT; ++i)
      if (strcmp(name, kOpts[i].name) == 0) return i;
  return -1;
}
}

namespace {
thread_local const int* t_call_opts = nullptr;
}
VlnceOptScope::VlnceOptScope(const int* per_call) : prev(t_call_opts) { t_call_opts = per_call; }
VlnceOptScope::~VlnceOptScope() { t_call_opts = prev; }

int vlnce_opt(int id) {
  if (t_call_opts && t_call_opts[id] >= 0) return t_call_opts[id];
  return g_opt[id].load(std::memory_order_relaxed);
}

extern "C" int vlnce_option_count(void) { return VLNCE_OPT_COUNT; }

extern "C" int vlnce_option_index(const char* name) { return opt_index(name); }

extern "C" int vlnce_set_option(const char* name, int value) {
  const int i = opt_index(name);
  if (i < 0) {
    vlnce_set_error("vlnce_set_option: unknown option '%s'", name ? name : "(null)");
    return 1;
  }
  g_opt[i].store(value, std::memory_order_relaxed);
  return 0;
}

extern "C" int vlnce_get_option(const char* name, int* value) {
  const int i = opt_index(name);
  if (i < 0 || !value) {
    vlnce_set_error("vlnce_get_option: unknown option '%s'", name ? name : "(null)");
    return 1;
  }
  *value = g_opt[i].load(std::memory_order_relaxed);
  return 0;
}

extern "C" int vlnce_option_default(const char* name, int* value) {
  const int i = opt_index(name);
  if (i < 0 || !value) {
    vlnce_set_error("vlnce_option_default: unknown option '%s'", name ? name : "(null)");
    return 1;
  }
  *value = kOpts[i].def;
  return 0;
}
```

### vln-ce_amd/csrc/common_opts.h

```cpp
#pragma once
#include "../../include/vlnce_hip.h"

void vlnce_set_error(const char* fmt, ...);

enum {
  VLNCE_OPT_CONV_MATH,
  VLNCE_OPT_P3,
  VLNCE_OPT_P3_TILE,
  VLNCE_OPT_S3,
  VLNCE_OPT_U3,
  VLNCE_OPT_U3_WAVES,
  VLNCE_OPT_X3_TILE,
  VLNCE_OPT_IGEMM_TILE,
  VLNCE_OPT_IGEMM_NOBUF,
  VLNCE_OPT_IGEMM_NO_SPLITK,
  VLNCE_OPT_WGRAD_TILE,
  VLNCE_OPT_ROLLOUT_ONE_XCD,
  VLNCE_OPT_M3,
  VLNCE_OPT_R3,
  VLNCE_OPT_S3_WGS,
  VLNCE_OPT_COUNT
};
int vlnce_opt(int id);

struct VlnceOptScope {
  explicit VlnceOptScope(const int* per_call);
  ~VlnceOptScope();
  const int* prev;
};
```

### vln-ce_amd/csrc/rnn_seq.hip

```cpp
#include "common.h"

namespace {

struct RnnSeqParams {
  const float* gi[2];
  const float* w_hh[2];
  const float* b_hh[2];
  float* out[2];
  float* h_final[2];
  float* gates[2];
  float* aux[2];
  const float* dout[2];
  const float* dh_final[2];
  float* dgi[2];
  float* dgh[2];
  const int* lengths;
  int B, L;
  float* seq[2];
  long seq_st, seq_sb;
  int self_zero;
  int w_plain;
};

__global__ __launch_bounds__(256) void dseq_to_time_major_kernel(const float* __restrict__ dseq, long st,
                                                                 long sb, float* __restrict__ dst, int dirs,
                                                                 int L, int B, int H) {
  const int h4 = H / 4;
  const long n = (long)dirs * L * B * h4;
  for (long i = (long)blockIdx.x * 256 + threadIdx.x; i < n; i += (long)gridDim.x * 256) {
    const int u4 = (int)(i % h4);
    long r = i / h4;
    const int b = (int)(r % B);
    r /= B;
    const int t = (int)(r % L);
    const int d = (int)(r / L);
    const float* src = dseq + (long)t * st + (long)b * sb + d * H + 4 * u4;
    f32x4 v = {src[0], src[1], src[2], src[3]};
    *reinterpret_cast<f32x4*>(dst + i * 4) = v;
  }
}

template <int NT>
__device__ __forceinline__ void zero_tails(float* __restrict__ base, long st, long sb, int width,
                                           const int* __restrict__ lengths, int b0, int B, int L,
                                           int tid) {
  for (int r = 0; r < 16; ++r) {
    const int b = b0 + r;
    if (b >= B) break;
    const int lb = min(max(lengths[b], 0), L);
    const int n = (L - lb) * width;
    for (int i = tid; i < n; i += NT) {
      const int q = i / width;
      base[(long)(lb + q) * st + (long)b * sb + (i - q * width)] = 0.f;
    }
  }
}

__device__ __forceinline__ float sigm(float x) {
  return __builtin_amdgcn_rcpf(1.f + __builtin_amdgcn_exp2f(-1.4426950408889634f * x));
}
__device__ __forceinline__ float tanh_fast(float x) {
  return 1.f - 2.f * __builtin_amdgcn_rcpf(__builtin_amdgcn_exp2f(2.8853900817779268f * x) + 1.f);
}

typedef __bf16 bf16x8 __attribute__((ext_vector_type(8)));
typedef unsigned u32x4r __attribute__((ext_vector_type(4)));
struct Planes3 {
  bf16x8 p[3];
};
__device__ __forceinline__ Planes3 split_planes(f32x4 lo4, f32x4 hi4) {
  const float x[8] = {lo4[0], lo4[1], lo4[2], lo4[3], hi4[0], hi4[1], hi4[2], hi4[3]};
  u32x4r h, m, l;
#pragma unroll
  for (int q = 0; q < 4; ++q) {
    const float x0 = x[2 * q], x1 = x[2 * q + 1];
    const float r0 = x0 - __uint_as_float(__float_as_uint(x0) & 0xffff0000u);
    const float r1 = x1 - __uint_as_float(__float_as_uint(x1) & 0xffff0000u);
    const float s0 = r0 - __uint_as_float(__float_as_uint(r0) & 0xffff0000u);
    const float s1 = r1 - __uint_as_float(__float_as_uint(r1) & 0xffff0000u);
    h[q] = __builtin_amdgcn_perm(__float_as_uint(x1), __float_as_uint(x0), 0x07060302u);
    m[q] = __builtin_amdgcn_perm(__float_as_uint(r1), __float_as_uint(r0), 0x07060302u);
    l[q] = __builtin_amdgcn_perm(__float_as_uint(s1), __float_as_uint(s0), 0x07060302u);
  }
  Planes3 o;
  o.p[0] = __builtin_bit_cast(bf16x8, h);
  o.p[1] = __builtin_bit_cast(bf16x8, m);
  o.p[2] = __builtin_bit_cast(bf16x8, l);
  return o;
}
__device__ __forceinline__ void split_scalar(float x, unsigned short (&o)[3]) {
  const unsigned xb = __float_as_uint(x);
  const float r = x - __uint_as_float(xb & 0xffff0000u);
  const unsigned rb = __float_as_uint(r);
  const float t = r - __uint_as_float(rb & 0xffff0000u);
  o[0] = (unsigned short)(xb >> 16);
  o[1] = (unsigned short)(rb >> 16);
  o[2] = (unsigned short)(__float_as_uint(t) >> 16);
}
constexpr int X3_PA[6] = {2, 0, 1, 1, 0, 0};
constexpr int X3_PB[6] = {0, 2, 1, 0, 1, 0};

template <int KIND, int H, int NW>
__global__ __launch_bounds__(NW * 64) void rnn_seq_fwd_kernel(RnnSeqParams p) {
  constexpr int G = KIND == 0 ? 4 : 3;
  constexpr int NTW = H / (NW * 16);
  static_assert(NTW >= 1, "units per wave");
  constexpr int KS = H / 32;
  constexpr int LDHB = H + 16;
  __shared__ __attribute__((aligned(16))) unsigned short h_pl[2][3][16][LDHB];
  constexpr int KL = (KIND == 0 && H == 128) ? 3 : 0;
  __shared__ __attribute__((aligned(16))) bf16x8 w_lds[KL > 0 ? KL : 1][3][NW * 64];
  const int d = blockIdx.y;
  const int b0 = blockIdx.x * 16;
  const int tid = threadIdx.x, lane = tid & 63, wave = tid >> 6;
  const int l15 = lane & 15, quad = lane >> 4;
  const bool reverse = d == 1;
  const float* __restrict__ gi = p.gi[d];
  const float* __restrict__ W = p.w_hh[d];
  const int B = p.B, L = p.L;
  if (p.self_zero) {
    zero_tails<NW * 64>(p.out[d], (long)B * H, H, H, p.lengths, b0, B, L, tid);
    if (p.seq[d]) zero_tails<NW * 64>(p.seq[d], p.seq_st, p.seq_sb, H, p.lengths, b0, B, L, tid);
  }

  int len[4];
#pragma unroll
  for (int r = 0; r < 4; ++r) {
    const int b = b0 + quad * 4 + r;
    len[r] = b < B ? p.lengths[b] : 0;
  }
  int Lt = max(max(len[0], len[1]), max(len[2], len[3]));
  Lt = max(Lt, __shfl_xor(Lt, 16, 64));
  Lt = max(Lt, __shfl_xor(Lt, 32, 64));
  Lt = min(Lt, L);
  Planes3 wp[G][NTW][KS];
  float bias[G][NTW];
#pragma unroll
  for (int gt = 0; gt < G; ++gt)
#pragma unroll
    for (int nt = 0; nt < NTW; ++nt) {
      const int n = gt * H + wave * (H / NW) + nt * 16 + l15;
      bias[gt][nt] = p.b_hh[d][n];
#pragma unroll
      for (int ks = 0; ks < KS; ++ks) {
        const float* w8 = W + (long)n * H + 32 * ks + 8 * quad;
        wp[gt][nt][ks] = split_planes(*reinterpret_cast<const f32x4*>(w8),
                                      *reinterpret_cast<const f32x4*>(w8 + 4));
        if (KL > 0 && gt == G - 1 && nt == 0 && ks >= KS - KL) {
#pragma unroll
          for (int q = 0; q < 3; ++q) w_lds[ks - (KS - KL)][q][tid] = wp[gt][nt][ks].p[q];
        }
      }
    }
  float hreg[NTW][4], creg[NTW][4];
#pragma unroll
  for (int nt = 0; nt < NTW; ++nt)
#pragma unroll
    for (int r = 0; r < 4; ++r) hreg[nt][r] = creg[nt][r] = 0.f;
  for (int i = tid; i < 3 * 16 * LDHB; i += NW * 64) (&h_pl[0][0][0][0])[i] = 0;
  __syncthreads();

  float gx[G][NTW][4];
  auto fetch_into = [&](int s, float (&dst)[G][NTW][4]) {
#pragma unroll
    for (int r = 0; r < 4; ++r) {
      const bool active = s < len[r];
      const int tt = reverse ? len[r] - 1 - s : s;
      const int b = b0 + quad * 4 + r;
      const float* row = gi + ((long)tt * B + b) * (G * H);
#pragma unroll
      for (int nt = 0; nt < NTW; ++nt) {
        const int u = wave * (H / NW) + nt * 16 + l15;
#pragma unroll
        for (int gt = 0; gt < G; ++gt) dst[gt][nt][r] = active ? row[gt * H + u] : 0.f;
      }
    }
  };
  auto fetch = [&](int s) { fetch_into(s, gx); };
  fetch(0);

#ifdef RNN_SEQ_DBG_TIME
  long long f_m = 0, f_g = 0, f_b = 0;
#endif
  for (int s = 0; s < Lt; ++s) {
#ifdef RNN_SEQ_DBG_TIME
    const long long f_t0 = clock64();
#endif
    const int cur = s & 1;
    f32x4 acc[G][NTW];
    float xn[NTW][4];
#pragma unroll
    for (int r = 0; r < 4; ++r)
#pragma unroll
      for (int nt = 0; nt < NTW; ++nt)
#pragma unroll
        for (int gt = 0; gt < G; ++gt) {
          const float x = gx[gt][nt][r];
          if (KIND == 1 && gt == 2) {
            xn[nt][r] = x;
            acc[gt][nt][r] = bias[gt][nt];
          } else {
            acc[gt][nt][r] = x + bias[gt][nt];
          }
        }
#pragma unroll
    for (int ks = 0; ks < KS; ++ks) {
      bf16x8 a[3];
#pragma unroll
      for (int q = 0; q < 3; ++q)
        a[q] = *reinterpret_cast<const bf16x8*>(&h_pl[cur][q][l15][32 * ks + 8 * quad]);
      Planes3 wl;
      const bool from_lds = KL > 0 && ks >= KS - KL;
      if (from_lds) {
#pragma unroll
        for (int q = 0; q < 3; ++q) wl.p[q] = w_lds[KL > 0 ? ks - (KS - KL) : 0][q][tid];
      }
#pragma unroll
      for (int q = 0; q < 6; ++q)
#pragma unroll
        for (int gt = 0; gt < G; ++gt)
#pragma unroll
          for (int nt = 0; nt < NTW; ++nt) {
            const bf16x8 wb = (from_lds && gt == G - 1 && nt == 0) ? wl.p[X3_PB[q]]
                                                                   : wp[gt][nt][ks].p[X3_PB[q]];
            acc[gt][nt] = __builtin_amdgcn_mfma_f32_16x16x32_bf16(a[X3_PA[q]], wb, acc[gt][nt], 0, 0, 0);
          }
    }
    fetch(s + 1);
#ifdef RNN_SEQ_DBG_TIME
    const long long f_t1 = clock64();
#endif
#pragma unroll
    for (int r = 0; r < 4; ++r) {
      const bool active = s < len[r];
      const int tt = reverse ? len[r] - 1 - s : s;
      const int b = b0 + quad * 4 + r;
      const int row_i = quad * 4 + r;
#pragma unroll
      for (int nt = 0; nt < NTW; ++nt) {
        const int u = wave * (H / NW) + nt * 16 + l15;
        float hnew;
        if (KIND == 0) {
          const float ig = sigm(acc[0][nt][r]), fg = sigm(acc[1][nt][r]);
          const float gg = tanh_fast(acc[2][nt][r]), og = sigm(acc[3][nt][r]);
          const float cn = fg * creg[nt][r] + ig * gg;
          hnew = og * tanh_fast(cn);
          if (active) {
            creg[nt][r] = cn;
            if (p.gates[d]) {
              float* gs = p.gates[d] + ((long)tt * B + b) * (G * H);
              gs[u] = ig;
              gs[H + u] = fg;
              gs[2 * H + u] = gg;
              gs[3 * H + u] = og;
              p.aux[d][((long)tt * B + b) * H + u] = cn;
            }
          }
        } else {
          const float rg = sigm(acc[0][nt][r]), zg = sigm(acc[1][nt][r]);
          const float hn = acc[2][nt][r];
          const float ng = tanh_fast(xn[nt][r] + rg * hn);
          hnew = (1.f - zg) * ng + zg * hreg[nt][r];
          if (active && p.gates[d]) {
            float* gs = p.gates[d] + ((long)tt * B + b) * (G * H);
            gs[u] = rg;
            gs[H + u] = zg;
            gs[2 * H + u] = ng;
            p.aux[d][((long)tt * B + b) * H + u] = hn;
          }
        }
        if (active) {
          hreg[nt][r] = hnew;
          p.out[d][((long)tt * B + b) * H + u] = hnew;
          if (p.seq[d]) p.seq[d][(long)tt * p.seq_st + (long)b * p.seq_sb + u] = hnew;
        }
        unsigned short hw[3];
        split_scalar(hreg[nt][r], hw);
#pragma unroll
        for (int q = 0; q < 3; ++q) h_pl[cur ^ 1][q][row_i][u] = hw[q];
      }
    }
#ifdef RNN_SEQ_DBG_TIME
    const long long f_t2 = clock64();
#endif
    __syncthreads();
#ifdef RNN_SEQ_DBG_TIME
    const long long f_t3 = clock64();
    f_m += f_t1 - f_t0;
    f_g += f_t2 - f_t1;
    f_b += f_t3 - f_t2;
#endif
  }
#ifdef RNN_SEQ_DBG_TIME
  if (blockIdx.x == 0 && blockIdx.y == 0 && (tid == 0 || tid == 64 * (NW - 1)))
    printf("rnn_seq_fwd wave %d: %d steps; per step: init+fetch+reads+MFMA %lld, gates+stores+LDS write %lld, "
           "barrier %lld cycles\n", wave, Lt, f_m / Lt, f_g / Lt, f_b / Lt);
#endif
#pragma unroll
  for (int r = 0; r < 4; ++r) {
    const int b = b0 + quad * 4 + r;
    if (b < B)
#pragma unroll
      for (int nt = 0; nt < NTW; ++nt)
        p.h_final[d][(long)b * H + wave * (H / NW) + nt * 16 + l15] = hreg[nt][r];
  }
}

template <int KIND, int H, int NW>
__global__ __launch_bounds__(NW * 64) void rnn_seq_bwd_kernel(RnnSeqParams p) {
  constexpr int G = KIND == 0 ? 4 : 3;
  constexpr int NTW = H / (NW * 16);
  constexpr int GH = G * H;
  constexpr int KS = GH / 32;
  constexpr int LDGB = GH + 16;
  static_assert(NTW >= 1, "units per wave");
  __shared__ __attribute__((aligned(16))) unsigned short dg_pl[3][16][LDGB];
  constexpr int KL = (KIND == 0 && H == 128) ? 4 : 0;
  __shared__ __attribute__((aligned(16))) bf16x8 w_lds[KL > 0 ? KL : 1][3][NW * 64];
  const int d = blockIdx.y;
  const int b0 = blockIdx.x * 16;
  const int tid = threadIdx.x, lane = tid & 63, wave = tid >> 6;
  const int l15 = lane & 15, quad = lane >> 4;
  const bool reverse = d == 1;
  const float* __restrict__ WT = p.w_hh[d];
  const int B = p.B, L = p.L;
  if (p.self_zero) {
    zero_tails<NW * 64>(p.dgi[d], (long)B * GH, GH, GH, p.lengths, b0, B, L, tid);
    if (KIND == 1) zero_tails<NW * 64>(p.dgh[d], (long)B * GH, GH, GH, p.lengths, b0, B, L, tid);
  }

  int len[4];
#pragma unroll
  for (int r = 0; r < 4; ++r) {
    const int b = b0 + quad * 4 + r;
    len[r] = b < B ? p.lengths[b] : 0;
  }
  int Lt = max(max(len[0], len[1]), max(len[2], len[3]));
  Lt = max(Lt, __shfl_xor(Lt, 16, 64));
  Lt = max(Lt, __shfl_xor(Lt, 32, 64));
  Lt = min(Lt, L);
  Planes3 wt[NTW][KS];
#pragma unroll
  for (int nt = 0; nt < NTW; ++nt) {
    const int n = wave * (H / NW) + nt * 16 + l15;
#pragma unroll
    for (int ks = 0; ks < KS; ++ks) {
      f32x4 lo4, hi4;
      if (p.w_plain) {
        const float* wk = WT + (long)(32 * ks + 8 * quad) * H + n;
#pragma unroll
        for (int i = 0; i < 4; ++i) {
          lo4[i] = wk[(long)i * H];
          hi4[i] = wk[(long)(i + 4) * H];
        }
      } else {
        const float* w8 = WT + (long)n * GH + 32 * ks + 8 * quad;
        lo4 = *reinterpret_cast<const f32x4*>(w8);
        hi4 = *reinterpret_cast<const f32x4*>(w8 + 4);
      }
      wt[nt][ks] = split_planes(lo4, hi4);
      if (KL > 0 && nt == 0 && ks >= KS - KL) {
#pragma unroll
        for (int q = 0; q < 3; ++q) w_lds[ks - (KS - KL)][q][tid] = wt[nt][ks].p[q];
      }
    }
  }
  float dh[NTW][4], dc[NTW][4];
#pragma unroll
  for (int nt = 0; nt < NTW; ++nt)
#pragma unroll
    for (int r = 0; r < 4; ++r) {
      const int b = b0 + quad * 4 + r;
      const int u = wave * (H / NW) + nt * 16 + l15;
      dh[nt][r] = (p.dh_final[d] && b < B) ? p.dh_final[d][(long)b * H + u] : 0.f;
      dc[nt][r] = 0.f;
    }

  float pg[G][NTW][4], pa[NTW][4], pa_prev[NTW][4], pd[NTW][4];
  auto fetch_row = [&](int s, int r, float (&g_)[G][NTW][4], float (&a_)[NTW][4], float (&d_)[NTW][4]) {
    {
      const bool active = s >= 0 && s < len[r];
      const int tt = reverse ? len[r] - 1 - s : s;
      const int b = b0 + quad * 4 + r;
      const long base = ((long)tt * B + b);
#pragma unroll
      for (int nt = 0; nt < NTW; ++nt) {
        const int u = wave * (H / NW) + nt * 16 + l15;
#pragma unroll
        for (int gt = 0; gt < G; ++gt) g_[gt][nt][r] = active ? p.gates[d][base * GH + gt * H + u] : 0.f;
        a_[nt][r] = active ? p.aux[d][base * H + u] : 0.f;
        d_[nt][r] = (active && p.dout[d]) ? p.dout[d][base * H + u] : 0.f;
      }
    }
  };
  auto fetch = [&](int s, float (&g_)[G][NTW][4], float (&a_)[NTW][4], float (&d_)[NTW][4]) {
#pragma unroll
    for (int r = 0; r < 4; ++r) fetch_row(s, r, g_, a_, d_);
  };
  auto fetch_prev_row = [&](int s, int r, float (&a_)[NTW][4]) {
    {
      const bool active = s >= 0 && s < len[r];
      const int tt = reverse ? len[r] - 1 - s : s;
      const int b = b0 + quad * 4 + r;
#pragma unroll
      for (int nt = 0; nt < NTW; ++nt) {
        const int u = wave * (H / NW) + nt * 16 + l15;
        const float* src = KIND == 0 ? p.aux[d] : p.out[d];
        a_[nt][r] = active ? src[((long)tt * B + b) * H + u] : 0.f;
      }
    }
  };
  auto fetch_prev = [&](int s, float (&a_)[NTW][4]) {
#pragma unroll
    for (int r = 0; r < 4; ++r) fetch_prev_row(s, r, a_);
  };
  fetch(Lt - 1, pg, pa, pd);
  fetch_prev(Lt - 2, pa_prev);

#ifdef RNN_SEQ_DBG_TIME
  long long d_a = 0, d_b1 = 0, d_m = 0, d_b2 = 0;
#endif
  for (int s = Lt - 1; s >= 0; --s) {
#ifdef RNN_SEQ_DBG_TIME
    const long long d_t0 = clock64();
#endif
    float keep_z[NTW][4];
    float cg[G][NTW][4], ca[NTW][4], cprev[NTW][4], cd[NTW][4];
#pragma unroll
    for (int r = 0; r < 4; ++r)
#pragma unroll
      for (int nt = 0; nt < NTW; ++nt) {
#pragma unroll
        for (int gt = 0; gt < G; ++gt) cg[gt][nt][r] = pg[gt][nt][r];
        ca[nt][r] = pa[nt][r];
        cprev[nt][r] = pa_prev[nt][r];
        cd[nt][r] = pd[nt][r];
      }
    fetch(s - 1, pg, pa, pd);
    fetch_prev(s - 2, pa_prev);
#pragma unroll
    for (int r = 0; r < 4; ++r) {
      const bool active = s < len[r];
      const int tt = reverse ? len[r] - 1 - s : s;
      const int b = b0 + quad * 4 + r;
      const int row_i = quad * 4 + r;
      const long base = ((long)tt * B + b);
#pragma unroll
      for (int nt = 0; nt < NTW; ++nt) {
        const int u = wave * (H / NW) + nt * 16 + l15;
        float dpre[G];
#pragma unroll
        for (int gt = 0; gt < G; ++gt) dpre[gt] = 0.f;
        float dgh_n = 0.f;
        keep_z[nt][r] = 0.f;
        if (active) {
          const float dht = dh[nt][r] + cd[nt][r];
          if (KIND == 0) {
            const float ig = cg[0][nt][r], fg = cg[1][nt][r], gg = cg[2][nt][r], og = cg[3][nt][r];
            const float c = ca[nt][r];
            const float cp = cprev[nt][r];
            const float tc = tanh_fast(c);
            const float dct = dc[nt][r] + dht * og * (1.f - tc * tc);
            dpre[0] = dct * gg * ig * (1.f - ig);
            dpre[1] = dct * cp * fg * (1.f - fg);
            dpre[2] = dct * ig * (1.f - gg * gg);
            dpre[3] = dht * tc * og * (1.f - og);
            dc[nt][r] = dct * fg;
          } else {
            const float rg = cg[0][nt][r], zg = cg[1][nt][r], ng = cg[2][nt][r];
            const float hn = ca[nt][r];
            const float hp = cprev[nt][r];
            const float dn = dht * (1.f - zg);
            const float dz = dht * (hp - ng);
            const float dnp = dn * (1.f - ng * ng);
            dpre[0] = dnp * hn * rg * (1.f - rg);
            dpre[1] = dz * zg * (1.f - zg);
            dpre[2] = dnp;
            dgh_n = dnp * rg;
            keep_z[nt][r] = dht * zg;
          }
          float* dgi = p.dgi[d] + base * GH;
#pragma unroll
          for (int gt = 0; gt < G; ++gt) dgi[gt * H + u] = dpre[gt];
          if (KIND == 1) {
            float* dgh = p.dgh[d] + base * GH;
            dgh[u] = dpre[0];
            dgh[H + u] = dpre[1];
            dgh[2 * H + u] = dgh_n;
          }
        }
#pragma unroll
        for (int gt = 0; gt < G; ++gt) {
          unsigned short dw[3];
          split_scalar((KIND == 1 && gt == 2) ? dgh_n : dpre[gt], dw);
#pragma unroll
          for (int q = 0; q < 3; ++q) dg_pl[q][row_i][gt * H + u] = dw[q];
        }
      }
    }
#ifdef RNN_SEQ_DBG_TIME
    const long long d_t1 = clock64();
#endif
    __syncthreads();
#ifdef RNN_SEQ_DBG_TIME
    const long long d_t2 = clock64();
#endif
    f32x4 acc[NTW];
#pragma unroll
    for (int nt = 0; nt < NTW; ++nt) acc[nt] = f32x4{0.f, 0.f, 0.f, 0.f};
#pragma unroll
    for (int ks = 0; ks < KS; ++ks) {
      bf16x8 a[3];
#pragma unroll
      for (int q = 0; q < 3; ++q)
        a[q] = *reinterpret_cast<const bf16x8*>(&dg_pl[q][l15][32 * ks + 8 * quad]);
      Planes3 wl;
      const bool from_lds = KL > 0 && ks >= KS - KL;
      if (from_lds) {
#pragma unroll
        for (int q = 0; q < 3; ++q) wl.p[q] = w_lds[KL > 0 ? ks - (KS - KL) : 0][q][tid];
      }
#pragma unroll
      for (int q = 0; q < 6; ++q)
#pragma unroll
        for (int nt = 0; nt < NTW; ++nt) {
          const bf16x8 wb = (from_lds && nt == 0) ? wl.p[X3_PB[q]] : wt[nt][ks].p[X3_PB[q]];
          acc[nt] = __builtin_amdgcn_mfma_f32_16x16x32_bf16(a[X3_PA[q]], wb, acc[nt], 0, 0, 0);
        }
    }
#pragma unroll
    for (int r = 0; r < 4; ++r) {
      const bool active = s < len[r];
      if (active)
#pragma unroll
        for (int nt = 0; nt < NTW; ++nt) dh[nt][r] = acc[nt][r] + keep_z[nt][r];
    }
#ifdef RNN_SEQ_DBG_TIME
    const long long d_t3 = clock64();
#endif
    __syncthreads();
#ifdef RNN_SEQ_DBG_TIME
    const long long d_t4 = clock64();
    d_a += d_t1 - d_t0;
    d_b1 += d_t2 - d_t1;
    d_m += d_t3 - d_t2;
    d_b2 += d_t4 - d_t3;
#endif
  }
#ifdef RNN_SEQ_DBG_TIME
  if (blockIdx.x == 0 && blockIdx.y == 0 && (tid == 0 || tid == 64 * (NW - 1)))
    printf("rnn_seq_bwd wave %d: %d steps; per step: gates+LDS write %lld, barrier %lld, reads+MFMA %lld, "
           "barrier %lld cycles\n", wave, Lt, d_a / Lt, d_b1 / Lt, d_m / Lt, d_b2 / Lt);
#endif
}

template <int KIND>
int launch_fwd(const RnnSeqParams& p, int H, int dirs, hipStream_t s) {
  dim3 grid(ceil_div(p.B, 16), dirs);
  if (H == 64)
    hipLaunchKernelGGL((rnn_seq_fwd_kernel<KIND, 64, 4>), grid, dim3(256), 0, s, p);
  else if (H == 128)
    hipLaunchKernelGGL((rnn_seq_fwd_kernel<KIND, 128, 8>), grid, dim3(512), 0, s, p);
  else
    return 1;
  return 0;
}
template <int KIND>
int launch_bwd(const RnnSeqParams& p, int H, int dirs, hipStream_t s) {
  dim3 grid(ceil_div(p.B, 16), dirs);
  if (H == 64)
    hipLaunchKernelGGL((rnn_seq_bwd_kernel<KIND, 64, 4>), grid, dim3(256), 0, s, p);
  else if (H == 128)
    hipLaunchKernelGGL((rnn_seq_bwd_kernel<KIND, 128, 8>), grid, dim3(512), 0, s, p);
  else
    return 1;
  return 0;
}

}

extern "C" int vlnce_rnn_seq_supported(int kind, int H) {
  return (kind == 0 || kind == 1) && (H == 64 || H == 128);
}

extern "C" int vlnce_rnn_seq_fwd(int kind, int dirs, const float* const* gi,
                                 const float* const* w_hh, const float* const* b_hh,
                                 const int* lengths, float* const* out, float* const* h_final,
                                 float* const* gates_save, float* const* aux_save, int B, int L,
                                 int H, vlnce_stream_t stream) {
  VLNCE_CHECK_ARG(gi && w_hh && b_hh && lengths && out && h_final, "rnn_seq_fwd: null argument");
  VLNCE_CHECK_ARG(dirs == 1 || dirs == 2, "rnn_seq_fwd: dirs must be 1 or 2");
  VLNCE_CHECK_ARG(vlnce_rnn_seq_supported(kind, H), "rnn_seq_fwd: unsupported kind/H (%d,%d)", kind, H);
  VLNCE_CHECK_ARG(B > 0 && L > 0, "rnn_seq_fwd: bad shape");
  RnnSeqParams p{};
  for (int d = 0; d < dirs; ++d) {
    p.gi[d] = gi[d];
    p.w_hh[d] = w_hh[d];
    p.b_hh[d] = b_hh[d];
    p.out[d] = out[d];
    p.h_final[d] = h_final[d];
    p.gates[d] = gates_save ? gates_save[d] : nullptr;
    p.aux[d] = aux_save ? aux_save[d] : nullptr;
    VLNCE_CHECK_ARG((p.gates[d] == nullptr) == (p.aux[d] == nullptr),
                    "rnn_seq_fwd: gates_save and aux_save come together");
  }
  p.lengths = lengths;
  p.B = B;
  p.L = L;
  hipStream_t s = reinterpret_cast<hipStream_t>(stream);
  const int rc = kind == 0 ? launch_fwd<0>(p, H, dirs, s) : launch_fwd<1>(p, H, dirs, s);
  VLNCE_CHECK_ARG(rc == 0, "rnn_seq_fwd: no kernel for H=%d", H);
  VLNCE_CHECK_LAUNCH("rnn_seq_fwd");
  return 0;
}

extern "C" int vlnce_rnn_seq_bwd(int kind, int dirs, const float* const* w_hh_t,
                                 const int* lengths, const float* const* out,
                                 const float* const* gates_save, const float* const* aux_save,
                                 const float* const* dout, const float* const* dh_final,
                                 float* const* dgi, float* const* dgh, int B, int L, int H,
                                 vlnce_stream_t stream) {
  VLNCE_CHECK_ARG(w_hh_t && lengths && out && gates_save && aux_save && dgi,
                  "rnn_seq_bwd: null argument");
  VLNCE_CHECK_ARG(dirs == 1 || dirs == 2, "rnn_seq_bwd: dirs must be 1 or 2");
  VLNCE_CHECK_ARG(vlnce_rnn_seq_supported(kind, H), "rnn_seq_bwd: unsupported kind/H (%d,%d)", kind, H);
  VLNCE_CHECK_ARG(kind == 0 || dgh, "rnn_seq_bwd: GRU needs dgh");
  RnnSeqParams p{};
  for (int d = 0; d < dirs; ++d) {
    p.w_hh[d] = w_hh_t[d];
    p.out[d] = const_cast<float*>(out[d]);
    p.gates[d] = const_cast<float*>(gates_save[d]);
    p.aux[d] = const_cast<float*>(aux_save[d]);
    p.dout[d] = dout ? dout[d] : nullptr;
    p.dh_final[d] = dh_final ? dh_final[d] : nullptr;
    p.dgi[d] = dgi[d];
    p.dgh[d] = dgh ? dgh[d] : nullptr;
  }
  p.lengths = lengths;
  p.B = B;
  p.L = L;
  hipStream_t s = reinterpret_cast<hipStream_t>(stream);
  const int rc = kind == 0 ? launch_bwd<0>(p, H, dirs, s) : launch_bwd<1>(p, H, dirs, s);
  VLNCE_CHECK_ARG(rc == 0, "rnn_seq_bwd: no kernel for H=%d", H);
  VLNCE_CHECK_LAUNCH("rnn_seq_bwd");
  return 0;
}


extern "C" int vlnce_rnn_seq_fwd2(int kind, int dirs, const float* const* gi,
                                  const float* const* w_hh, const float* const* b_hh,
                                  const int* lengths, float* const* out_tm, float* seq,
                                  long seq_st, long seq_sb, float* const* h_final,
                                  float* const* gates_save, float* const* aux_save, int B, int L,
                                  int H, vlnce_stream_t stream) {
  VLNCE_CHECK_ARG(gi && w_hh && b_hh && lengths && out_tm && h_final, "rnn_seq_fwd2: null argument");
  VLNCE_CHECK_ARG(dirs == 1 || dirs == 2, "rnn_seq_fwd2: dirs must be 1 or 2");
  VLNCE_CHECK_ARG(vlnce_rnn_seq_supported(kind, H), "rnn_seq_fwd2: unsupported kind/H (%d,%d)", kind, H);
  VLNCE_CHECK_ARG(B > 0 && L > 0, "rnn_seq_fwd2: bad shape");
  VLNCE_CHECK_ARG(!seq || (seq_st > 0 && seq_sb > 0), "rnn_seq_fwd2: seq needs its strides");
  RnnSeqParams p{};
  for (int d = 0; d < dirs; ++d) {
    p.gi[d] = gi[d];
    p.w_hh[d] = w_hh[d];
    p.b_hh[d] = b_hh[d];
    p.out[d] = out_tm[d];
    p.seq[d] = seq ? seq + (long)d * H : nullptr;
    p.h_final[d] = h_final[d];
    p.gates[d] = gates_save ? gates_save[d] : nullptr;
    p.aux[d] = aux_save ? aux_save[d] : nullptr;
    VLNCE_CHECK_ARG((p.gates[d] == nullptr) == (p.aux[d] == nullptr),
                    "rnn_seq_fwd2: gates_save and aux_save come together");
  }
  p.seq_st = seq_st;
  p.seq_sb = seq_sb;
  p.self_zero = 1;
  p.lengths = lengths;
  p.B = B;
  p.L = L;
  hipStream_t s = reinterpret_cast<hipStream_t>(stream);
  const int rc = kind == 0 ? launch_fwd<0>(p, H, dirs, s) : launch_fwd<1>(p, H, dirs, s);
  VLNCE_CHECK_ARG(rc == 0, "rnn_seq_fwd2: no kernel for H=%d", H);
  VLNCE_CHECK_LAUNCH("rnn_seq_fwd2");
  return 0;
}

extern "C" int vlnce_rnn_seq_bwd2(int kind, int dirs, const float* const* w_hh, const int* lengths,
                                  const float* const* out_tm, const float* const* gates_save,
                                  const float* const* aux_save, const float* dseq, long dseq_st,
                                  long dseq_sb, float* dout_ws, const float* const* dh_final,
                                  float* const* dgi, float* const* dgh, int B, int L, int H,
                                  vlnce_stream_t stream) {
  VLNCE_CHECK_ARG(w_hh && lengths && out_tm && gates_save && aux_save && dgi,
                  "rnn_seq_bwd2: null argument");
  VLNCE_CHECK_ARG(dirs == 1 || dirs == 2, "rnn_seq_bwd2: dirs must be 1 or 2");
  VLNCE_CHECK_ARG(vlnce_rnn_seq_supported(kind, H), "rnn_seq_bwd2: unsupported kind/H (%d,%d)", kind, H);
  VLNCE_CHECK_ARG(kind == 0 || dgh, "rnn_seq_bwd2: GRU needs dgh");
  VLNCE_CHECK_ARG(!dseq || (dseq_st > 0 && dseq_sb > 0), "rnn_seq_bwd2: dseq needs its strides");
  VLNCE_CHECK_ARG(!dseq || dout_ws, "rnn_seq_bwd2: dseq needs the dirs*L*B*H workspace");
  hipStream_t s = reinterpret_cast<hipStream_t>(stream);
  if (dseq) {
    const long n4 = (long)dirs * L * B * (H / 4);
    const int grid = (int)((n4 + 255) / 256 > 2048 ? 2048 : (n4 + 255) / 256);
    hipLaunchKernelGGL(dseq_to_time_major_kernel, dim3(grid), dim3(256), 0, s, dseq, dseq_st, dseq_sb,
                       dout_ws, dirs, L, B, H);
    VLNCE_CHECK_LAUNCH("rnn_seq_bwd2 (output gradient to time-major)");
  }
  RnnSeqParams p{};
  for (int d = 0; d < dirs; ++d) {
    p.w_hh[d] = w_hh[d];
    p.out[d] = const_cast<float*>(out_tm[d]);
    p.gates[d] = const_cast<float*>(gates_save[d]);
    p.aux[d] = const_cast<float*>(aux_save[d]);
    p.dout[d] = dseq ? dout_ws + (long)d * L * B * H : nullptr;
    p.dh_final[d] = dh_final ? dh_final[d] : nullptr;
    p.dgi[d] = dgi[d];
    p.dgh[d] = dgh ? dgh[d] : nullptr;
  }
  p.self_zero = 1;
  p.w_plain = 1;
  p.lengths = lengths;
  p.B = B;
  p.L = L;
  const int rc = kind == 0 ? launch_bwd<0>(p, H, dirs, s) : launch_bwd<1>(p, H, dirs, s);
  VLNCE_CHECK_ARG(rc == 0, "rnn_seq_bwd2: no kernel for H=%d", H);
  VLNCE_CHECK_LAUNCH("rnn_seq_bwd2");
  return 0;
}

extern "C" int vlnce_rnn_seq_wgrad(int kind, int dirs, int first_dir, const float* const* dgi,
                                   const float* const* dgh, const float* const* out_tm,
                                   const float* x_tm, int ldx, int E, const float* const* w_ih,
                                   float* const* dw_ih, float* const* dw_hh, float* const* db_ih,
                                   float* const* db_hh, float* dx_tm, int B, int L, int H,
                                   vlnce_stream_t stream) {
  VLNCE_CHECK_ARG(dgi && out_tm && x_tm && dw_ih && dw_hh && db_ih && db_hh,
                  "rnn_seq_wgrad: null argument");
  VLNCE_CHECK_ARG(dirs == 1 || dirs == 2, "rnn_seq_wgrad: dirs must be 1 or 2");
  VLNCE_CHECK_ARG((first_dir == 0 || first_dir == 1) && first_dir + dirs <= 2,
                  "rnn_seq_wgrad: first_dir + dirs must stay within the two directions");
  VLNCE_CHECK_ARG(kind == 0 || dgh, "rnn_seq_wgrad: GRU needs dgh");
  VLNCE_CHECK_ARG(!dx_tm || w_ih, "rnn_seq_wgrad: dx_tm needs w_ih");
  const int GH = (kind == 0 ? 4 : 3) * H;
  const long rows = (long)L * B;
  VLNCE_CHECK_ARG(B > 0 && L > 0 && E > 0 && ldx >= E && rows < 0x7fffffffL, "rnn_seq_wgrad: bad shape");
  hipStream_t s = reinterpret_cast<hipStream_t>(stream);
  for (int d = 0; d < dirs; ++d) {
    const float* dGh = kind == 1 ? dgh[d] : dgi[d];
    if (L > 1) {
      const bool reverse = first_dir + d == 1;
      const float* dG_s = reverse ? dGh : dGh + (long)B * GH;
      const float* h_s = reverse ? out_tm[d] + (long)B * H : out_tm[d];
      int rc = vlnce_gemm(dG_s, GH, 1, h_s, H, 1, dw_hh[d], H, GH, H, (int)((long)(L - 1) * B), nullptr, stream);
      if (rc != 0) return rc;
    } else {
      vlnce_zero(dw_hh[d], GH, H, H, s);
    }
    int rc = vlnce_colsum(dGh, GH, (int)rows, GH, db_hh[d], 0, stream);
    if (rc != 0) return rc;
    rc = vlnce_gemm(dgi[d], GH, 1, x_tm, ldx, 1, dw_ih[d], E, GH, E, (int)rows, nullptr, stream);
    if (rc != 0) return rc;
    if (db_ih[d] != db_hh[d]) {
      rc = vlnce_colsum(dgi[d], GH, (int)rows, GH, db_ih[d], 0, stream);
      if (rc != 0) return rc;
    }
    if (dx_tm) {
      vlnce_epilogue e{};
      e.accumulate = d > 0;
      rc = vlnce_gemm(dgi[d], GH, 0, w_ih[d], E, 1, dx_tm, E, (int)rows, E, GH, &e, stream);
      if (rc != 0) return rc;
    }
  }
  return 0;
}
```

### vln-ce_amd/ops.py

```python
import os

import torch
import torch.nn.functional as F
from torch.autograd import Function

from . import _lib

ACT_NONE, ACT_RELU, ACT_SIGMOID, ACT_TANH = 0, 1, 2, 3


def L():
    return _lib.get_lib()


def _f32c(t):
    if t.dtype != torch.float32:
        t = t.float()
    return t if t.is_contiguous() else t.contiguous()


def _rows2d(t):
    if t.dim() != 2 or t.stride(1) != 1 or (t.size(0) > 1 and t.stride(0) < t.size(1)):
        t = t.reshape(-1, t.size(-1)).contiguous()
    ld = t.stride(0) if t.size(0) > 1 else t.size(1)
# ... 730 lines not shown
        return out, None


def mask_rows(x, mask_u8):
    return MaskRowsFn.apply(x, mask_u8)


class SelectRowsFn(Function):

    @staticmethod
    def forward(ctx, mask_u8, a, b_):
        ref = a if a is not None else b_
        a = _f32c(a) if a is not None else None
        b_ = _f32c(b_) if b_ is not None else None
        B, H = ref.shape
        out = torch.empty((B, H), device=ref.device, dtype=torch.float32)
        L().select_rows(mask_u8, a, b_, out, B, H)
        ctx.save_for_backward(mask_u8)
        ctx.has = (a is not None, b_ is not None)
        return out

    @staticmethod
    def backward(ctx, g):
        (m,) = ctx.saved_tensors
        g = _f32c(g)
        B, H = g.shape
        ga = gb = None
        if ctx.has[0] and ctx.needs_input_grad[1]:
            ga = torch.empty_like(g)
            L().select_rows(m, g, None, ga, B, H)
        if ctx.has[1] and ctx.needs_input_grad[2]:
            gb = torch.empty_like(g)
            L().select_rows(m, None, g, gb, B, H)
        return None, ga, gb


def select_rows(mask_u8, a, b_):
    return SelectRowsFn.apply(mask_u8, a, b_)


class MeanRowsFn(Function):

    @staticmethod
    def forward(ctx, x):
        x = _f32c(x)
        B, P, Cc = x.shape
        y = torch.empty((B, Cc), device=x.device, dtype=torch.float32)
        L().mean_rows(x, y, B, P, Cc)
        ctx.P = P
        return y

    @staticmethod
    def backward(ctx, g):
        return (g / ctx.P).unsqueeze(1).expand(-1, ctx.P, -1)


def mean_rows(x):
    return MeanRowsFn.apply(x)


class GRUGatesFn(Function):

    @staticmethod
    def forward(ctx, gi, gh, h_prev):
        gi, gh, h_prev = _f32c(gi), _f32c(gh), _f32c(h_prev)
        B, H = h_prev.shape
        h = torch.empty_like(h_prev)
        gates = torch.empty((B, 3 * H), device=h.device, dtype=torch.float32)
        hn = torch.empty_like(h_prev)
        L().gru_gates_fwd(gi, gh, h_prev, None, h, gates, hn, B, H)
        ctx.save_for_backward(gates, hn, h_prev)
        return h

    @staticmethod
    def backward(ctx, dh):
        gates, hn, h_prev = ctx.saved_tensors
        B, H = h_prev.shape
        dh = _f32c(dh)
        dgi = torch.empty_like(gates)
        dgh = torch.empty_like(gates)
        dhp = torch.empty_like(h_prev)
        L().gru_gates_bwd(dh, gates, hn, h_prev, None, dgi, dgh, dhp, B, H)
        return dgi, dgh, dhp


class LSTMGatesFn(Function):

    @staticmethod
    def forward(ctx, gi, gh, c_prev):
        gi, gh, c_prev = _f32c(gi), _f32c(gh), _f32c(c_prev)
        B, H = c_prev.shape
        h = torch.empty_like(c_prev)
        c = torch.empty_like(c_prev)
        gates = torch.empty((B, 4 * H), device=h.device, dtype=torch.float32)
        L().lstm_gates_fwd(gi, gh, c_prev, None, h, c, gates, B, H)
        ctx.save_for_backward(gates, c_prev, c)
        return h, c

    @staticmethod
    def backward(ctx, dh, dc):
        gates, c_prev, c = ctx.saved_tensors
        B, H = c_prev.shape
        dh = _f32c(dh) if dh is not None else None
        dc = _f32c(dc) if dc is not None else None
        dg = torch.empty_like(gates)
        dcp = torch.empty_like(c_prev)
        L().lstm_gates_bwd(dh, dc, gates, c_prev, c, None, dg, dcp, B, H)
        return dg, dg, dcp


def gru_cell(x_gates, h_prev, w_hh, b_hh):
    gh = linear(h_prev, w_hh, b_hh)
    return GRUGatesFn.apply(x_gates, gh, h_prev)


def lstm_cell(x_gates, h_prev, c_prev, w_hh, b_hh):
    gh = linear(h_prev, w_hh, b_hh)
    return LSTMGatesFn.apply(x_gates, gh, c_prev)


_ROLLOUT_WS = {}


def _rollout_workspace(dev, nbytes):
    if dev.type == "cuda" and torch.cuda.is_current_stream_capturing():
        return torch.empty(nbytes, dtype=torch.uint8, device=dev)
    key = (str(dev), torch.cuda.current_stream(dev).cuda_stream if dev.type == "cuda" else 0)
    w = _ROLLOUT_WS.get(key)
    if w is None or w.numel() < nbytes:
        w = _ROLLOUT_WS[key] = torch.empty(max(nbytes, 1 << 19), dtype=torch.uint8, device=dev)
    return w


class MaskedRNNSeqFn(Function):

    @staticmethod
    def forward(ctx, lstm, gi, h0, c0, mask, w_hh, b_hh):
        lib = L()
        gi, h0, w_hh = _f32c(gi), _f32c(h0), _f32c(w_hh)
        N, H = h0.shape
        T = gi.size(0) // N
        GH = gi.size(1)
        dev = gi.device
        hp = torch.empty((T, N, H), device=dev, dtype=torch.float32)
        out = torch.empty((T, N, H), device=dev, dtype=torch.float32)
        gates = torch.empty((T, N, GH), device=dev, dtype=torch.float32)
        aux = torch.empty((T, N, H), device=dev, dtype=torch.float32)
        gh = torch.empty((N, GH), device=dev, dtype=torch.float32)
        gi3, m2 = gi.view(T, N, GH), mask.view(T, N)
        h, c = h0, (_f32c(c0) if lstm else None)
        b_hh = _f32c(b_hh)
        supported = getattr(lib, "lstm_rollout_supported", None) if lstm else lib.gru_rollout_supported
        ctx.rollout = T > 1 and supported is not None and bool(supported(N, H))
        if ctx.rollout:
            ctx.lstm, ctx.dims = lstm, (T, N, H, GH)
            if lstm:
                ws = _rollout_workspace(dev, lib.lstm_rollout_workspace_bytes(N, H))
                lib.lstm_rollout_fwd(gi3, h0, c, m2.contiguous(), w_hh, b_hh, hp, out, gates, aux,
                                     ws, T, N, H)
                ctx.save_for_backward(hp, gates, aux, m2, w_hh, c)
                return out.view(T * N, H), out[T - 1], aux[T - 1]
            lib.gru_rollout_fwd(gi3, h0, m2.contiguous(), w_hh, b_hh, hp, out, gates, aux,
                                _rollout_workspace(dev, lib.gru_rollout_workspace_bytes(N, H)),
                                T, N, H)
            ctx.save_for_backward(hp, gates, aux, m2, w_hh, h0)
            return out.view(T * N, H), out[T - 1], out[T - 1]
        fused = lib.rnn_step_supported(N, H, lstm)
        for t in range(T):
            if fused:
                lib.rnn_step_fwd(lstm, gi3[t], h, c, m2[t], w_hh, b_hh, hp[t], out[t], aux[t],
                                 gates[t], N, H)
                if lstm:
                    c = aux[t]
                h = out[t]
                continue
            lib.mask_rows(h, m2[t], hp[t], N, H)
            lib.gemm(hp[t], H, 0, w_hh, H, 0, gh, GH, N, GH, H, shift=b_hh)
            if lstm:
                lib.lstm_gates_fwd(gi3[t], gh, c, m2[t], out[t], aux[t], gates[t], N, H)
                c = aux[t]
            else:
                lib.gru_gates_fwd(gi3[t], gh, hp[t], None, out[t], gates[t], aux[t], N, H)
            h = out[t]
        ctx.lstm, ctx.dims = lstm, (T, N, H, GH)
        ctx.save_for_backward(hp, gates, aux, m2, w_hh, _f32c(c0) if lstm else h0)
        return out.view(T * N, H), out[T - 1], (aux[T - 1] if lstm else out[T - 1])

    @staticmethod
    def backward(ctx, dout, dh_fin, dc_fin):
        lib = L()
        hp, gates, aux, m2, w_hh, c0 = ctx.saved_tensors
        T, N, H, GH = ctx.dims
        lstm = ctx.lstm
        dev = hp.device
        if ctx.rollout and lstm:
            dgi = torch.empty((T, N, GH), device=dev, dtype=torch.float32)
            dh0 = torch.empty((N, H), device=dev, dtype=torch.float32)
            dc0 = torch.empty((N, H), device=dev, dtype=torch.float32)
            lib.lstm_rollout_bwd(None if dout is None else _f32c(dout),
                                 None if dh_fin is None else _f32c(dh_fin),
                                 None if dc_fin is None else _f32c(dc_fin), gates, aux, hp, c0,
                                 m2.contiguous(), w_hh.t().contiguous(), dgi, dh0, dc0,
                                 _rollout_workspace(dev, lib.lstm_rollout_workspace_bytes(N, H)),
                                 T, N, H)
            dw = torch.empty_like(w_hh)
            lib.gemm(dgi.view(T * N, GH), GH, 1, hp.view(T * N, H), H, 1, dw, H, GH, H, T * N)
            db = torch.empty((GH,), device=dev, dtype=torch.float32)
            lib.colsum(dgi.view(T * N, GH), GH, T * N, GH, db, 0)
            return None, dgi.view(T * N, GH), dh0, dc0, None, dw, db
        if ctx.rollout:
            dgi = torch.empty((T, N, GH), device=dev, dtype=torch.float32)
            dgh = torch.empty_like(dgi)
            dh0 = torch.empty((N, H), device=dev, dtype=torch.float32)
            carry = None if dh_fin is None else _f32c(dh_fin)
            if dc_fin is not None:
                carry = _f32c(dc_fin) if carry is None else carry + dc_fin
            lib.gru_rollout_bwd(None if dout is None else _f32c(dout), carry, gates, aux, hp,
                                m2.contiguous(), w_hh.t().contiguous(), dgi, dgh, dh0,
                                _rollout_workspace(dev, lib.gru_rollout_workspace_bytes(N, H)),
                                T, N, H)
            dw = torch.empty_like(w_hh)
            lib.gemm(dgh.view(T * N, GH), GH, 1, hp.view(T * N, H), H, 1, dw, H, GH, H, T * N)
            db = torch.empty((GH,), device=dev, dtype=torch.float32)
            lib.colsum(dgh.view(T * N, GH), GH, T * N, GH, db, 0)
            return None, dgi.view(T * N, GH), dh0, None, None, dw, db
        dout = _f32c(dout).view(T, N, H)
        mf = m2.to(torch.float32).unsqueeze(-1)
        dgi = torch.empty((T, N, GH), device=dev, dtype=torch.float32)
        dgh = dgi if lstm else torch.empty_like(dgi)
        carry = torch.zeros((N, H), device=dev, dtype=torch.float32) if dh_fin is None \
            else _f32c(dh_fin).clone()
        if not lstm and dc_fin is not None:
            carry = carry + dc_fin
        dc = None
        if lstm:
            dc = torch.zeros((N, H), device=dev, dtype=torch.float32) if dc_fin is None \
                else _f32c(dc_fin).clone()
        dh_t = torch.empty((N, H), device=dev, dtype=torch.float32)
        acc = torch.empty((N, H), device=dev, dtype=torch.float32)
        dc_prev = torch.empty((N, H), device=dev, dtype=torch.float32) if lstm else None
        fused = lib.rnn_step_supported(N, H, lstm)
        w_hh_t = w_hh.t().contiguous() if fused else None
        for t in range(T - 1, -1, -1):
            if fused:
                c_prev = (aux[t - 1] if t > 0 else c0) if lstm else None
                lib.rnn_step_bwd(lstm, dout[t], carry, dc, gates[t], aux[t], hp[t], c_prev, m2[t],
                                 w_hh_t, dgi[t], dgh[t], acc, dc_prev, N, H)
                if lstm:
                    dc, dc_prev = dc_prev, dc
                continue
            torch.add(dout[t], carry, out=dh_t)
            if lstm:
                c_prev = aux[t - 1] if t > 0 else c0
                lib.lstm_gates_bwd(dh_t, dc, gates[t], c_prev, aux[t], m2[t], dgi[t], dc_prev,
                                   N, H)
                dc, dc_prev = dc_prev, dc
                lib.gemm(dgi[t], GH, 0, w_hh, H, 1, acc, H, N, H, GH)
            else:
                lib.gru_gates_bwd(dh_t, gates[t], aux[t], hp[t], None, dgi[t], dgh[t], acc, N, H)
                lib.gemm(dgh[t], GH, 0, w_hh, H, 1, acc, H, N, H, GH, accumulate=1)
            torch.mul(acc, mf[t], out=carry)
        dw = torch.empty_like(w_hh)
        lib.gemm(dgh.view(T * N, GH), GH, 1, hp.view(T * N, H), H, 1, dw, H, GH, H, T * N)
        db = torch.empty((GH,), device=dev, dtype=torch.float32)
        lib.colsum(dgh.view(T * N, GH), GH, T * N, GH, db, 0)
        dc0 = dc if lstm else None
        return None, dgi.view(T * N, GH), carry, dc0, None, dw, db


class RNNLayerFn(Function):

    @staticmethod
    def forward(ctx, kind, save, lengths, dirs, B, Lm, x_tm, *params):
        x_tm, ldx = _rows2d(_f32c(x_tm) if x_tm.dtype != torch.float32 else x_tm)
        E = x_tm.size(1)
        w_ih = [_f32c(params[4 * d]) for d in range(dirs)]
        b_ih = [params[4 * d + 1] for d in range(dirs)]
        w_hh = [_f32c(params[4 * d + 2]) for d in range(dirs)]
        b_hh = [_f32c(params[4 * d + 3]) for d in range(dirs)]
        GH, H = w_hh[0].shape
        dev = x_tm.device
        lib = L()
        rows = Lm * B
        gis = []
        for d in range(dirs):
            gi = torch.empty((rows, GH), device=dev, dtype=torch.float32)
            if not _planes_gemm(x_tm, ldx, w_ih[d], gi, b_ih[d]):
                lib.gemm(x_tm, ldx, 0, w_ih[d], E, 0, gi, GH, rows, GH, E, shift=b_ih[d])
            gis.append(gi.view(Lm, B, GH))

        def new(*shape):
            return torch.empty(shape, device=dev, dtype=torch.float32)

        out_tm = [new(Lm, B, H) for _ in range(dirs)]
        seq = new(B, Lm, dirs * H)
        hfin = [new(B, H) for _ in range(dirs)]
        gates = aux = None
        if save:
            gates = [new(Lm, B, GH) for _ in range(dirs)]
            aux = [new(Lm, B, H) for _ in range(dirs)]
        lib.rnn_seq_fwd2(kind, dirs, gis, w_hh, b_hh, lengths, out_tm, seq, dirs * H, Lm * dirs * H,
                         hfin, gates, aux, B, Lm, H)
        ctx.cfg = (kind, dirs, Lm, B, H, GH, E, ldx)
        ctx.set_materialize_grads(False)
        if save:
            ctx.save_for_backward(lengths, x_tm, *w_ih, *w_hh, *out_tm, *gates, *aux)
        return (seq, *hfin)

    @staticmethod
    def backward(ctx, dseq, *dhf):
        kind, dirs, Lm, B, H, GH, E, ldx = ctx.cfg
        sv = ctx.saved_tensors
        lengths, x_tm = sv[0], sv[1]
        w_ih, w_hh = sv[2:2 + dirs], sv[2 + dirs:2 + 2 * dirs]
        out_tm = sv[2 + 2 * dirs:2 + 3 * dirs]
        gates = sv[2 + 3 * dirs:2 + 4 * dirs]
        aux = sv[2 + 4 * dirs:2 + 5 * dirs]
        dev = x_tm.device
        st = sb = 0
        if dseq is not None:
            if (dseq.dtype != torch.float32 or dseq.stride(2) != 1 or dseq.stride(0) <= 0
                    or dseq.stride(1) <= 0):
                dseq = _f32c(dseq)
            sb, st = dseq.stride(0), dseq.stride(1)
        dhf = [(_f32c(g) if g is not None else None) for g in dhf[:dirs]]

        def new(*shape):
            return torch.empty(shape, device=dev, dtype=torch.float32)

        dgi = [new(Lm, B, GH) for _ in range(dirs)]
        dgh = [new(Lm, B, GH) for _ in range(dirs)] if kind == 1 else None
        lib = L()
        ws = new(dirs, Lm, B, H) if dseq is not None else None
        lib.rnn_seq_bwd2(kind, dirs, list(w_hh), lengths, list(out_tm), list(gates), list(aux), dseq,
                         st, sb, ws, dhf, dgi, dgh, B, Lm, H)
        dw_ih = [new(GH, E) for _ in range(dirs)]
        dw_hh = [new(GH, H) for _ in range(dirs)]
        db_ih = [new(GH) for _ in range(dirs)]
        db_hh = [new(GH) for _ in range(dirs)]
        need_dx = ctx.needs_input_grad[6]
        dx = new(Lm * B, E) if need_dx else None
        from .streams import BranchStreams

        if (dirs == 2 and Lm * B >= 2048 and BranchStreams.enabled(dev)
                and os.environ.get("VLNCE_RNN_WGRAD_STREAMS", "1") != "0"):
            cur = torch.cuda.current_stream(dev)
            side = BranchStreams()._stream(1, dev)
            if side is cur:
                side = BranchStreams()._stream(2, dev)
            dx1 = new(Lm * B, E) if need_dx else None
            fork = torch.cuda.Event()
            fork.record(cur)
            side.wait_event(fork)
            with torch.cuda.stream(side):
                lib.rnn_seq_wgrad(kind, 1, dgi[1:], dgh[1:] if dgh else None, list(out_tm[1:]), x_tm, ldx, E,
                                  list(w_ih[1:]), dw_ih[1:], dw_hh[1:], db_ih[1:], db_hh[1:], dx1, B, Lm,
                                  H, first_dir=1)
                done = torch.cuda.Event()
                done.record(side)
            lib.rnn_seq_wgrad(kind, 1, dgi[:1], dgh[:1] if dgh else None, list(out_tm[:1]), x_tm, ldx, E,
                              list(w_ih[:1]), dw_ih[:1], dw_hh[:1], db_ih[:1], db_hh[:1], dx, B, Lm, H)
            cur.wait_event(done)
            if need_dx:
                dx.add_(dx1)
        else:
            lib.rnn_seq_wgrad(kind, dirs, dgi, dgh, list(out_tm), x_tm, ldx, E, list(w_ih), dw_ih, dw_hh,
                              db_ih, db_hh, dx, B, Lm, H)
        res = [None, None, None, None, None, None, dx]
        for d in range(dirs):
            res += [dw_ih[d], db_ih[d], dw_hh[d], db_hh[d]]
        return tuple(res)


def rnn_layer(kind, lengths_i32, x_tm, B, Lm, per_direction, need_grad):
    flat = [t for quad in per_direction for t in quad]
    res = RNNLayerFn.apply(kind, bool(need_grad), lengths_i32, len(per_direction), B, Lm, x_tm, *flat)
    return res[0], list(res[1:])
```

Baseline: 8403.

## Add fp16 three-product split-precision path for sequence RNN recurrent matmuls

Adds an rnn_math option and an fp16x3 split-plane MFMA path for the sequence GRU/LSTM forward and backward kernels. Weights get per-row power-of-two scaling and are split into two fp16 planes, so each product needs three MFMAs instead of six bf16 ones, with some syncthreads dropped. By default this path is used only for H=128, or for GRU in backward. The trade is less range and precision margin in exchange for fewer matrix ops on the serial recurrent critical path.

```diff
diff --git a/include/vlnce_hip.h b/include/vlnce_hip.h
--- a/include/vlnce_hip.h
+++ b/include/vlnce_hip.h
@@ -321,23 +321,23 @@
 int vlnce_rnn_seq_fwd(int kind, int dirs, const float* const* gi, const float* const* w_hh,
                       const float* const* b_hh, const int* lengths, float* const* out,
                       float* const* h_final, float* const* gates_save, float* const* aux_save,
-                      int B, int L, int H, vlnce_stream_t stream);
+                      int B, int L, int H, const int* options, vlnce_stream_t stream);
 int vlnce_rnn_seq_bwd(int kind, int dirs, const float* const* w_hh_t, const int* lengths,
                       const float* const* out, const float* const* gates_save,
                       const float* const* aux_save, const float* const* dout,
                       const float* const* dh_final, float* const* dgi, float* const* dgh,
-                      int B, int L, int H, vlnce_stream_t stream);
+                      int B, int L, int H, const int* options, vlnce_stream_t stream);
 int vlnce_rnn_seq_fwd2(int kind, int dirs, const float* const* gi, const float* const* w_hh,
                        const float* const* b_hh, const int* lengths, float* const* out_tm,
                        float* seq, long seq_st, long seq_sb, float* const* h_final,
                        float* const* gates_save, float* const* aux_save, int B, int L, int H,
-                       vlnce_stream_t stream);
+                       const int* options, vlnce_stream_t stream);
 int vlnce_rnn_seq_bwd2(int kind, int dirs, const float* const* w_hh, const int* lengths,
                        const float* const* out_tm, const float* const* gates_save,
                        const float* const* aux_save, const float* dseq, long dseq_st, long dseq_sb,
                        float* dout_ws ,
                        const float* const* dh_final, float* const* dgi, float* const* dgh,
-                       int B, int L, int H, vlnce_stream_t stream);
+                       int B, int L, int H, const int* options, vlnce_stream_t stream);
 int vlnce_rnn_seq_wgrad(int kind, int dirs, int first_dir, const float* const* dgi, const float* const* dgh,
                         const float* const* out_tm, const float* x_tm, int ldx, int E,
                         const float* const* w_ih, float* const* dw_ih, float* const* dw_hh,
diff --git a/vln-ce_amd/_lib.py b/vln-ce_amd/_lib.py
--- a/vln-ce_amd/_lib.py
+++ b/vln-ce_amd/_lib.py
@@ -196,15 +196,15 @@
     "vlnce_maxpool3x3s2_bwd": (_I, [_P, _P, _P, _I, _I, _I, _I, _I, _I, _P]),
     "vlnce_adaptive_avgpool_bwd": (_I, [_P, _P, _I, _I, _I, _I, _I, _I, _P]),
     "vlnce_rnn_seq_supported": (_I, [_I, _I]),
-    "vlnce_rnn_seq_fwd": (_I, [_I, _I, _P, _P, _P, _P, _P, _P, _P, _P, _I, _I, _I, _P]),
-    "vlnce_rnn_seq_bwd": (_I, [_I, _I, _P, _P, _P, _P, _P, _P, _P, _P, _P, _I, _I, _I, _P]),
+    "vlnce_rnn_seq_fwd": (_I, [_I, _I, _P, _P, _P, _P, _P, _P, _P, _P, _I, _I, _I, _P, _P]),
+    "vlnce_rnn_seq_bwd": (_I, [_I, _I, _P, _P, _P, _P, _P, _P, _P, _P, _P, _I, _I, _I, _P, _P]),
     "vlnce_option_count": (_I, []),
     "vlnce_option_index": (_I, [C.c_char_p]),
     "vlnce_linear_rows_supported": (_I, [_I, _I, _I]),
     "vlnce_linear_rows_fwd": (_I, [_P, _I, _P, _I, _P, _I, _P, _I, _I, _I, _I, _P]),
     "vlnce_linear_rows_bwd": (_I, [_P, _I, _P, _I, _P, _I, _P, _I, _I, _P, _P, _P, _I, _I, _I, _P]),
-    "vlnce_rnn_seq_fwd2": (_I, [_I, _I, _P, _P, _P, _P, _P, _P, _L, _L, _P, _P, _P, _I, _I, _I, _P]),
-    "vlnce_rnn_seq_bwd2": (_I, [_I, _I, _P, _P, _P, _P, _P, _P, _L, _L, _P, _P, _P, _P, _I, _I, _I, _P]),
+    "vlnce_rnn_seq_fwd2": (_I, [_I, _I, _P, _P, _P, _P, _P, _P, _L, _L, _P, _P, _P, _I, _I, _I, _P, _P]),
+    "vlnce_rnn_seq_bwd2": (_I, [_I, _I, _P, _P, _P, _P, _P, _P, _L, _L, _P, _P, _P, _P, _I, _I, _I, _P, _P]),
     "vlnce_rnn_seq_wgrad": (_I, [_I, _I, _I, _P, _P, _P, _P, _I, _I, _P, _P, _P, _P, _P, _P, _I, _I, _I, _P]),
     "vlnce_group_norm_small": (_I, [_P, _I, _I, _I, _I, _P, _P, _F, _P, _I, _P, _P]),
     "vlnce_gru_rollout_supported": (_I, [_I, _I]),
@@ -306,7 +306,7 @@
 
     name = "hip"
 
-    ABI = 150
+    ABI = 151
 
     def __init__(self, path=LIB_PATH):
         self.dll = load_cdll(path)
@@ -321,7 +321,7 @@
 
     OPTION_NAMES = ("conv_math", "p3", "p3_tile", "s3", "u3", "u3_waves", "x3_tile", "igemm_tile",
                     "igemm_nobuf", "igemm_no_splitk", "wgrad_tile", "rollout_one_xcd", "m3", "r3",
-                    "s3_wgs")
+                    "s3_wgs", "rnn_math")
 
     def _options_from_env(self):
         for name in self.OPTION_NAMES:
@@ -330,6 +330,8 @@
                 continue
             if name == "conv_math":
                 v = {"f32": 0, "0": 0, "bf16": 1, "1": 1, "f16": 2, "2": 2}.get(v.strip().lower(), v)
+            elif name == "rnn_math":
+                v = {"bf16": 1, "1": 1, "f16": 2, "2": 2, "3": 3}.get(v.strip().lower(), v)
             elif name in ("igemm_nobuf", "igemm_no_splitk"):
                 v = 0 if v in ("", "0") else 1
             try:
@@ -376,7 +378,8 @@
         self._check(self.dll.vlnce_option_default(name.encode(), C.byref(v)), "vlnce_option_default")
         return v.value
 
-    PER_LAUNCH = ("conv_math", "p3", "p3_tile", "s3", "u3", "u3_waves", "x3_tile", "m3", "r3", "s3_wgs")
+    PER_LAUNCH = ("conv_math", "p3", "p3_tile", "s3", "u3", "u3_waves", "x3_tile", "m3", "r3", "s3_wgs",
+                  "rnn_math")
 
     def _launch_options(self, overrides):
         if not overrides:
@@ -877,21 +880,25 @@
     def rnn_seq_supported(self, kind, H):
         return bool(self.dll.vlnce_rnn_seq_supported(kind, H))
 
+    def _rnn_options(self, options):
+        opts = self._launch_options(options if options is not None else getattr(self._tls, "scoped", None))
+        return C.cast(opts, C.c_void_p) if opts is not None else None
+
     def rnn_seq_fwd(self, kind, dirs, gi, w_hh, b_hh, lengths, out, h_final, gates_save, aux_save,
-                    B, Lm, H):
+                    B, Lm, H, options=None):
         pa = self._parr
         self._check(self.dll.vlnce_rnn_seq_fwd(
             kind, dirs, pa(gi, dirs), pa(w_hh, dirs), pa(b_hh, dirs), _ptr(lengths), pa(out, dirs),
-            pa(h_final, dirs), pa(gates_save, dirs), pa(aux_save, dirs), B, Lm, H, _stream()),
-            "vlnce_rnn_seq_fwd")
+            pa(h_final, dirs), pa(gates_save, dirs), pa(aux_save, dirs), B, Lm, H,
+            self._rnn_options(options), _stream()), "vlnce_rnn_seq_fwd")
 
     def rnn_seq_bwd(self, kind, dirs, w_hh_t, lengths, out, gates_save, aux_save, dout, dh_final,
-                    dgi, dgh, B, Lm, H):
+                    dgi, dgh, B, Lm, H, options=None):
         pa = self._parr
         self._check(self.dll.vlnce_rnn_seq_bwd(
             kind, dirs, pa(w_hh_t, dirs), _ptr(lengths), pa(out, dirs), pa(gates_save, dirs),
             pa(aux_save, dirs), pa(dout, dirs), pa(dh_final, dirs), pa(dgi, dirs), pa(dgh, dirs),
-            B, Lm, H, _stream()), "vlnce_rnn_seq_bwd")
+            B, Lm, H, self._rnn_options(options), _stream()), "vlnce_rnn_seq_bwd")
 
     def linear_rows_supported(self, M, N, K):
         return bool(self.dll.vlnce_linear_rows_supported(M, N, K))
@@ -906,20 +913,21 @@
                                                    _stream()), "vlnce_linear_rows_bwd")
 
     def rnn_seq_fwd2(self, kind, dirs, gi, w_hh, b_hh, lengths, out_tm, seq, seq_st, seq_sb, h_final,
-                     gates_save, aux_save, B, Lm, H):
+                     gates_save, aux_save, B, Lm, H, options=None):
         pa = self._parr
         self._check(self.dll.vlnce_rnn_seq_fwd2(
             kind, dirs, pa(gi, dirs), pa(w_hh, dirs), pa(b_hh, dirs), _ptr(lengths), pa(out_tm, dirs),
             _ptr(seq), seq_st, seq_sb, pa(h_final, dirs), pa(gates_save, dirs), pa(aux_save, dirs),
-            B, Lm, H, _stream()), "vlnce_rnn_seq_fwd2")
+            B, Lm, H, self._rnn_options(options), _stream()), "vlnce_rnn_seq_fwd2")
 
     def rnn_seq_bwd2(self, kind, dirs, w_hh, lengths, out_tm, gates_save, aux_save, dseq, dseq_st,
-                     dseq_sb, dout_ws, dh_final, dgi, dgh, B, Lm, H):
+                     dseq_sb, dout_ws, dh_final, dgi, dgh, B, Lm, H, options=None):
         pa = self._parr
         self._check(self.dll.vlnce_rnn_seq_bwd2(
             kind, dirs, pa(w_hh, dirs), _ptr(lengths), pa(out_tm, dirs), pa(gates_save, dirs),
             pa(aux_save, dirs), _ptr(dseq), dseq_st, dseq_sb, _ptr(dout_ws), pa(dh_final, dirs),
-            pa(dgi, dirs), pa(dgh, dirs), B, Lm, H, _stream()), "vlnce_rnn_seq_bwd2")
+            pa(dgi, dirs), pa(dgh, dirs), B, Lm, H, self._rnn_options(options), _stream()),
+            "vlnce_rnn_seq_bwd2")
 
     def rnn_seq_wgrad(self, kind, dirs, dgi, dgh, out_tm, x_tm, ldx, E, w_ih, dw_ih, dw_hh, db_ih,
                       db_hh, dx_tm, B, Lm, H, first_dir=0):
diff --git a/vln-ce_amd/csrc/api.cpp b/vln-ce_amd/csrc/api.cpp
--- a/vln-ce_amd/csrc/api.cpp
+++ b/vln-ce_amd/csrc/api.cpp
@@ -16,7 +16,7 @@
 }
 
 extern "C" const char* vlnce_last_error(void) { return g_err; }
-extern "C" int vlnce_version(void) { return 150; }
+extern "C" int vlnce_version(void) { return 151; }
 
 namespace {
 struct OptDef {
@@ -27,10 +27,10 @@
     {"conv_math", 2},   {"p3", 2},          {"p3_tile", 0},         {"s3", 1},
     {"u3", 1},          {"u3_waves", 8},    {"x3_tile", 0},         {"igemm_tile", 0},
     {"igemm_nobuf", 0}, {"igemm_no_splitk", 0}, {"wgrad_tile", 64}, {"rollout_one_xcd", 0},
-    {"m3", 1},          {"r3", 1},          {"s3_wgs", 0},
+    {"m3", 1},          {"r3", 1},          {"s3_wgs", 0},          {"rnn_math", 2},
 };
 std::atomic<int> g_opt[VLNCE_OPT_COUNT] = {
-    {2}, {2}, {0}, {1}, {1}, {8}, {0}, {0}, {0}, {0}, {64}, {0}, {1}, {1}, {0},
+    {2}, {2}, {0}, {1}, {1}, {8}, {0}, {0}, {0}, {0}, {64}, {0}, {1}, {1}, {0}, {2},
 };
 int opt_index(const char* name) {
   if (name)
diff --git a/vln-ce_amd/csrc/common_opts.h b/vln-ce_amd/csrc/common_opts.h
--- a/vln-ce_amd/csrc/common_opts.h
+++ b/vln-ce_amd/csrc/common_opts.h
@@ -19,6 +19,7 @@
   VLNCE_OPT_M3,
   VLNCE_OPT_R3,
   VLNCE_OPT_S3_WGS,
+  VLNCE_OPT_RNN_MATH,
   VLNCE_OPT_COUNT
 };
 int vlnce_opt(int id);
diff --git a/vln-ce_amd/csrc/rnn_seq.hip b/vln-ce_amd/csrc/rnn_seq.hip
--- a/vln-ce_amd/csrc/rnn_seq.hip
+++ b/vln-ce_amd/csrc/rnn_seq.hip
@@ -1,6 +1,12 @@
 #include "common.h"
+#include "igemm_shared.h"
 
 namespace {
+
+using vlnce_detail::bf16x8;
+using vlnce_detail::f16x8;
+using vlnce_detail::MATH_BF16X6;
+using vlnce_detail::MATH_F16X3;
 
 struct RnnSeqParams {
   const float* gi[2];
@@ -63,7 +69,6 @@
   return 1.f - 2.f * __builtin_amdgcn_rcpf(__builtin_amdgcn_exp2f(2.8853900817779268f * x) + 1.f);
 }
 
-typedef __bf16 bf16x8 __attribute__((ext_vector_type(8)));
 typedef unsigned u32x4r __attribute__((ext_vector_type(4)));
 struct Planes3 {
   bf16x8 p[3];
@@ -100,16 +105,95 @@
 constexpr int X3_PA[6] = {2, 0, 1, 1, 0, 0};
 constexpr int X3_PB[6] = {0, 2, 1, 0, 1, 0};
 
-template <int KIND, int H, int NW>
+struct Pow2 {
+  float down, up;
+};
+__device__ __forceinline__ Pow2 pow2_of(unsigned abs_bits) {
+  unsigned be = abs_bits >> 23;
+  be = (be == 0 || be >= 255) ? 127u : min(max(be, 24u), 253u);
+  return Pow2{__uint_as_float((254u - be) << 23), __uint_as_float(be << 23)};
+}
+__device__ __forceinline__ unsigned abs_bits(float x) { return __float_as_uint(x) & 0x7fffffffu; }
+__device__ __forceinline__ unsigned wave_max_u32(unsigned v) {
+  v = max(v, (unsigned)__builtin_amdgcn_update_dpp(0, (int)v, 0xB1, 0xf, 0xf, false));
+  v = max(v, (unsigned)__builtin_amdgcn_update_dpp(0, (int)v, 0x4E, 0xf, 0xf, false));
+  v = max(v, (unsigned)__builtin_amdgcn_update_dpp(0, (int)v, 0x141, 0xf, 0xf, false));
+  v = max(v, (unsigned)__builtin_amdgcn_update_dpp(0, (int)v, 0x140, 0xf, 0xf, false));
+  return max(max((unsigned)__builtin_amdgcn_readlane((int)v, 0), (unsigned)__builtin_amdgcn_readlane((int)v, 16)),
+             max((unsigned)__builtin_amdgcn_readlane((int)v, 32), (unsigned)__builtin_amdgcn_readlane((int)v, 48)));
+}
+
+template <int MATH>
+struct RnnMath;
+template <>
+struct RnnMath<MATH_BF16X6> {
+  static constexpr int NA = 3, NB = 3, NP = 6;
+};
+template <>
+struct RnnMath<MATH_F16X3> {
+  static constexpr int NA = 2, NB = 2, NP = 3;
+};
+template <int MATH>
+struct WFrag {
+  bf16x8 p[RnnMath<MATH>::NB];
+};
+template <int MATH>
+__device__ __forceinline__ WFrag<MATH> split_frag(f32x4 lo4, f32x4 hi4, float scale) {
+  WFrag<MATH> o;
+  if constexpr (MATH == MATH_F16X3) {
+    const float x[8] = {lo4[0], lo4[1], lo4[2], lo4[3], hi4[0], hi4[1], hi4[2], hi4[3]};
+    u32x4r w0, w1;
+#pragma unroll
+    for (int q = 0; q < 4; ++q) {
+      unsigned w[2];
+      vlnce_detail::split_pair<MATH_F16X3>(x[2 * q] * scale, x[2 * q + 1] * scale, w);
+      w0[q] = w[0];
+      w1[q] = w[1];
+    }
+    o.p[0] = __builtin_bit_cast(bf16x8, w0);
+    o.p[1] = __builtin_bit_cast(bf16x8, w1);
+  } else {
+    const Planes3 t = split_planes(lo4, hi4);
+#pragma unroll
+    for (int q = 0; q < 3; ++q) o.p[q] = t.p[q];
+  }
+  return o;
+}
+__device__ __forceinline__ void f16x3_mfma(int q, const bf16x8 (&a)[2], const WFrag<MATH_F16X3>& b, f32x4& hi,
+                                           f32x4& lo) {
+  const f16x8 a1 = __builtin_bit_cast(f16x8, a[0]), a2 = __builtin_bit_cast(f16x8, a[1]);
+  const f16x8 b1 = __builtin_bit_cast(f16x8, b.p[0]), b2 = __builtin_bit_cast(f16x8, b.p[1]);
+  if (q == 0)
+    lo = __builtin_amdgcn_mfma_f32_16x16x32_f16(a2, b1, lo, 0, 0, 0);
+  else if (q == 1)
+    lo = __builtin_amdgcn_mfma_f32_16x16x32_f16(a1, b2, lo, 0, 0, 0);
+  else
+    hi = __builtin_amdgcn_mfma_f32_16x16x32_f16(a1, b1, hi, 0, 0, 0);
+}
+__device__ __forceinline__ void store_pair_f16(float v0, float v1, unsigned short* pl, int plane_stride, int pitch) {
+  unsigned w[2];
+  vlnce_detail::split_pair<MATH_F16X3>(v0, v1, w);
+#pragma unroll
+  for (int q = 0; q < 2; ++q) {
+    pl[q * plane_stride] = (unsigned short)(w[q] & 0xffffu);
+    pl[q * plane_stride + pitch] = (unsigned short)(w[q] >> 16);
+  }
+}
+constexpr float F16X3_POST = vlnce_detail::Planes<MATH_F16X3>::POST;
+
+template <int KIND, int H, int NW, int MATH>
 __global__ __launch_bounds__(NW * 64) void rnn_seq_fwd_kernel(RnnSeqParams p) {
   constexpr int G = KIND == 0 ? 4 : 3;
   constexpr int NTW = H / (NW * 16);
   static_assert(NTW >= 1, "units per wave");
   constexpr int KS = H / 32;
   constexpr int LDHB = H + 16;
-  __shared__ __attribute__((aligned(16))) unsigned short h_pl[2][3][16][LDHB];
-  constexpr int KL = (KIND == 0 && H == 128) ? 3 : 0;
-  __shared__ __attribute__((aligned(16))) bf16x8 w_lds[KL > 0 ? KL : 1][3][NW * 64];
+  constexpr int NA = RnnMath<MATH>::NA, NB = RnnMath<MATH>::NB, NP = RnnMath<MATH>::NP;
+  __shared__ __attribute__((aligned(16))) unsigned short h_pl[2][NA][16][LDHB];
+  constexpr int KL = (MATH == MATH_BF16X6 && KIND == 0 && H == 128) ? 3 : 0;
+  __shared__ __attribute__((aligned(16))) bf16x8 w_lds[KL > 0 ? KL : 1][NB][NW * 64];
+  constexpr bool F16 = MATH == MATH_F16X3;
+  __shared__ __attribute__((aligned(16))) f32x4 post_lds[F16 ? 2 : 1][F16 ? NTW : 1][F16 ? NW * 64 : 1];
   const int d = blockIdx.y;
   const int b0 = blockIdx.x * 16;
   const int tid = threadIdx.x, lane = tid & 63, wave = tid >> 6;
@@ -133,31 +217,62 @@
   Lt = max(Lt, __shfl_xor(Lt, 16, 64));
   Lt = max(Lt, __shfl_xor(Lt, 32, 64));
   Lt = min(Lt, L);
-  Planes3 wp[G][NTW][KS];
+  WFrag<MATH> wp[G][NTW][KS];
   float bias[G][NTW];
+  float wpost[G][NTW];
 #pragma unroll
   for (int gt = 0; gt < G; ++gt)
 #pragma unroll
     for (int nt = 0; nt < NTW; ++nt) {
       const int n = gt * H + wave * (H / NW) + nt * 16 + l15;
       bias[gt][nt] = p.b_hh[d][n];
+      f32x4 raw[KS][2];
 #pragma unroll
       for (int ks = 0; ks < KS; ++ks) {
         const float* w8 = W + (long)n * H + 32 * ks + 8 * quad;
-        wp[gt][nt][ks] = split_planes(*reinterpret_cast<const f32x4*>(w8),
-                                      *reinterpret_cast<const f32x4*>(w8 + 4));
+        raw[ks][0] = *reinterpret_cast<const f32x4*>(w8);
+        raw[ks][1] = *reinterpret_cast<const f32x4*>(w8 + 4);
+      }
+      Pow2 sc{1.f, 1.f};
+      if constexpr (MATH == MATH_F16X3) {
+        unsigned mb = 0;
+#pragma unroll
+        for (int ks = 0; ks < KS; ++ks)
+#pragma unroll
+          for (int i = 0; i < 4; ++i) mb = max(mb, max(abs_bits(raw[ks][0][i]), abs_bits(raw[ks][1][i])));
+        mb = max(mb, (unsigned)__shfl_xor((int)mb, 16, 64));
+        mb = max(mb, (unsigned)__shfl_xor((int)mb, 32, 64));
+        sc = pow2_of(mb);
+      }
+      wpost[gt][nt] = sc.up;
+#pragma unroll
+      for (int ks = 0; ks < KS; ++ks) {
+        wp[gt][nt][ks] = split_frag<MATH>(raw[ks][0], raw[ks][1], sc.down);
         if (KL > 0 && gt == G - 1 && nt == 0 && ks >= KS - KL) {
 #pragma unroll
-          for (int q = 0; q < 3; ++q) w_lds[ks - (KS - KL)][q][tid] = wp[gt][nt][ks].p[q];
+          for (int q = 0; q < NB; ++q) w_lds[ks - (KS - KL)][q][tid] = wp[gt][nt][ks].p[q];
         }
       }
     }
+  if constexpr (F16) {
+#pragma unroll
+    for (int nt = 0; nt < NTW; ++nt) {
+      f32x4 bv = {0.f, 0.f, 0.f, 0.f}, pv = bv;
+#pragma unroll
+      for (int gt = 0; gt < G; ++gt) {
+        bv[gt] = bias[gt][nt];
+        pv[gt] = wpost[gt][nt];
+      }
+      post_lds[0][nt][tid] = bv;
+      post_lds[1][nt][tid] = pv;
+    }
+  }
   float hreg[NTW][4], creg[NTW][4];
 #pragma unroll
   for (int nt = 0; nt < NTW; ++nt)
 #pragma unroll
     for (int r = 0; r < 4; ++r) hreg[nt][r] = creg[nt][r] = 0.f;
-  for (int i = tid; i < 3 * 16 * LDHB; i += NW * 64) (&h_pl[0][0][0][0])[i] = 0;
+  for (int i = tid; i < NA * 16 * LDHB; i += NW * 64) (&h_pl[0][0][0][0])[i] = 0;
   __syncthreads();
 
   float gx[G][NTW][4];
@@ -187,7 +302,7 @@
     const long long f_t0 = clock64();
 #endif
     const int cur = s & 1;
-    f32x4 acc[G][NTW];
+    f32x4 acc[G][NTW], lo[G][NTW];
     float xn[NTW][4];
 #pragma unroll
     for (int r = 0; r < 4; ++r)
@@ -196,37 +311,75 @@
 #pragma unroll
         for (int gt = 0; gt < G; ++gt) {
           const float x = gx[gt][nt][r];
-          if (KIND == 1 && gt == 2) {
-            xn[nt][r] = x;
-            acc[gt][nt][r] = bias[gt][nt];
+          if (KIND == 1 && gt == 2) xn[nt][r] = x;
+          if constexpr (MATH == MATH_F16X3) {
+            acc[gt][nt][r] = 0.f;
+            lo[gt][nt][r] = 0.f;
           } else {
-            acc[gt][nt][r] = x + bias[gt][nt];
+            acc[gt][nt][r] = (KIND == 1 && gt == 2) ? bias[gt][nt] : x + bias[gt][nt];
           }
         }
+    float ini[G][NTW][4];
+    if constexpr (F16) {
+#pragma unroll
+      for (int r = 0; r < 4; ++r)
+#pragma unroll
+        for (int nt = 0; nt < NTW; ++nt)
+#pragma unroll
+          for (int gt = 0; gt < G; ++gt) ini[gt][nt][r] = gx[gt][nt][r];
+      fetch(s + 1);
+    }
+    f32x4 bv[NTW], pv[NTW];
 #pragma unroll
     for (int ks = 0; ks < KS; ++ks) {
-      bf16x8 a[3];
-#pragma unroll
-      for (int q = 0; q < 3; ++q)
+      bf16x8 a[NA];
+#pragma unroll
+      for (int q = 0; q < NA; ++q)
         a[q] = *reinterpret_cast<const bf16x8*>(&h_pl[cur][q][l15][32 * ks + 8 * quad]);
-      Planes3 wl;
+      if constexpr (F16) {
+        if (ks == KS - 1) {
+#pragma unroll
+          for (int nt = 0; nt < NTW; ++nt) {
+            bv[nt] = post_lds[0][nt][tid];
+            pv[nt] = post_lds[1][nt][tid];
+          }
+        }
+      }
+      WFrag<MATH> wl;
       const bool from_lds = KL > 0 && ks >= KS - KL;
       if (from_lds) {
 #pragma unroll
-        for (int q = 0; q < 3; ++q) wl.p[q] = w_lds[KL > 0 ? ks - (KS - KL) : 0][q][tid];
-      }
-#pragma unroll
-      for (int q = 0; q < 6; ++q)
+        for (int q = 0; q < NB; ++q) wl.p[q] = w_lds[KL > 0 ? ks - (KS - KL) : 0][q][tid];
+      }
+#pragma unroll
+      for (int q = 0; q < NP; ++q)
 #pragma unroll
         for (int gt = 0; gt < G; ++gt)
 #pragma unroll
-          for (int nt = 0; nt < NTW; ++nt) {
-            const bf16x8 wb = (from_lds && gt == G - 1 && nt == 0) ? wl.p[X3_PB[q]]
-                                                                   : wp[gt][nt][ks].p[X3_PB[q]];
-            acc[gt][nt] = __builtin_amdgcn_mfma_f32_16x16x32_bf16(a[X3_PA[q]], wb, acc[gt][nt], 0, 0, 0);
+          for (int nt = 0; nt < NTW; ++nt)
+          {
+            if constexpr (MATH == MATH_F16X3) {
+              f16x3_mfma(q, a, wp[gt][nt][ks], acc[gt][nt], lo[gt][nt]);
+            } else {
+              const bf16x8 wb = (from_lds && gt == G - 1 && nt == 0) ? wl.p[X3_PB[q]]
+                                                                     : wp[gt][nt][ks].p[X3_PB[q]];
+              acc[gt][nt] = __builtin_amdgcn_mfma_f32_16x16x32_bf16(a[X3_PA[q]], wb, acc[gt][nt], 0, 0, 0);
+            }
           }
     }
-    fetch(s + 1);
+    if constexpr (F16) {
+#pragma unroll
+      for (int nt = 0; nt < NTW; ++nt)
+#pragma unroll
+        for (int r = 0; r < 4; ++r)
+#pragma unroll
+          for (int gt = 0; gt < G; ++gt) {
+            const float x0 = (KIND == 1 && gt == 2) ? bv[nt][gt] : ini[gt][nt][r] + bv[nt][gt];
+            acc[gt][nt][r] = fmaf(fmaf(lo[gt][nt][r], F16X3_POST, acc[gt][nt][r]), pv[nt][gt], x0);
+          }
+    } else {
+      fetch(s + 1);
+    }
 #ifdef RNN_SEQ_DBG_TIME
     const long long f_t1 = clock64();
 #endif
@@ -274,10 +427,14 @@
           p.out[d][((long)tt * B + b) * H + u] = hnew;
           if (p.seq[d]) p.seq[d][(long)tt * p.seq_st + (long)b * p.seq_sb + u] = hnew;
         }
-        unsigned short hw[3];
-        split_scalar(hreg[nt][r], hw);
-#pragma unroll
-        for (int q = 0; q < 3; ++q) h_pl[cur ^ 1][q][row_i][u] = hw[q];
+        if constexpr (MATH == MATH_BF16X6) {
+          unsigned short hw[3];
+          split_scalar(hreg[nt][r], hw);
+#pragma unroll
+          for (int q = 0; q < 3; ++q) h_pl[cur ^ 1][q][row_i][u] = hw[q];
+        } else if (r & 1) {
+          store_pair_f16(hreg[nt][r & ~1], hreg[nt][r], &h_pl[cur ^ 1][0][quad * 4 + (r & ~1)][u], 16 * LDHB, LDHB);
+        }
       }
     }
 #ifdef RNN_SEQ_DBG_TIME
@@ -306,17 +463,20 @@
   }
 }
 
-template <int KIND, int H, int NW>
+template <int KIND, int H, int NW, int MATH>
 __global__ __launch_bounds__(NW * 64) void rnn_seq_bwd_kernel(RnnSeqParams p) {
   constexpr int G = KIND == 0 ? 4 : 3;
   constexpr int NTW = H / (NW * 16);
   constexpr int GH = G * H;
   constexpr int KS = GH / 32;
   constexpr int LDGB = GH + 16;
+  constexpr int NA = RnnMath<MATH>::NA, NB = RnnMath<MATH>::NB, NP = RnnMath<MATH>::NP;
   static_assert(NTW >= 1, "units per wave");
-  __shared__ __attribute__((aligned(16))) unsigned short dg_pl[3][16][LDGB];
-  constexpr int KL = (KIND == 0 && H == 128) ? 4 : 0;
-  __shared__ __attribute__((aligned(16))) bf16x8 w_lds[KL > 0 ? KL : 1][3][NW * 64];
+  __shared__ __attribute__((aligned(16))) unsigned short dg_pl[NA][16][LDGB];
+  __shared__ __attribute__((aligned(16))) unsigned wave_max[8];
+  static_assert(NW <= 8 && NW % 4 == 0, "wave_max");
+  constexpr int KL = (MATH == MATH_BF16X6 && KIND == 0 && H == 128) ? 4 : 0;
+  __shared__ __attribute__((aligned(16))) bf16x8 w_lds[KL > 0 ? KL : 1][NB][NW * 64];
   const int d = blockIdx.y;
   const int b0 = blockIdx.x * 16;
   const int tid = threadIdx.x, lane = tid & 63, wave = tid >> 6;
@@ -339,13 +499,12 @@
   Lt = max(Lt, __shfl_xor(Lt, 16, 64));
   Lt = max(Lt, __shfl_xor(Lt, 32, 64));
   Lt = min(Lt, L);
-  Planes3 wt[NTW][KS];
+  WFrag<MATH> wt[NTW][KS];
+  float wpost[NTW];
 #pragma unroll
   for (int nt = 0; nt < NTW; ++nt) {
     const int n = wave * (H / NW) + nt * 16 + l15;
-#pragma unroll
-    for (int ks = 0; ks < KS; ++ks) {
-      f32x4 lo4, hi4;
+    auto load8 = [&](int ks, f32x4& lo4, f32x4& hi4) {
       if (p.w_plain) {
         const float* wk = WT + (long)(32 * ks + 8 * quad) * H + n;
 #pragma unroll
@@ -358,10 +517,30 @@
         lo4 = *reinterpret_cast<const f32x4*>(w8);
         hi4 = *reinterpret_cast<const f32x4*>(w8 + 4);
       }
-      wt[nt][ks] = split_planes(lo4, hi4);
+    };
+    Pow2 sc{1.f, 1.f};
+    if constexpr (MATH == MATH_F16X3) {
+      unsigned mb = 0;
+#pragma unroll
+      for (int ks = 0; ks < KS; ++ks) {
+        f32x4 lo4, hi4;
+        load8(ks, lo4, hi4);
+#pragma unroll
+        for (int i = 0; i < 4; ++i) mb = max(mb, max(abs_bits(lo4[i]), abs_bits(hi4[i])));
+      }
+      mb = max(mb, (unsigned)__shfl_xor((int)mb, 16, 64));
+      mb = max(mb, (unsigned)__shfl_xor((int)mb, 32, 64));
+      sc = pow2_of(mb);
+    }
+    wpost[nt] = sc.up;
+#pragma unroll
+    for (int ks = 0; ks < KS; ++ks) {
+      f32x4 lo4, hi4;
+      load8(ks, lo4, hi4);
+      wt[nt][ks] = split_frag<MATH>(lo4, hi4, sc.down);
       if (KL > 0 && nt == 0 && ks >= KS - KL) {
 #pragma unroll
-        for (int q = 0; q < 3; ++q) w_lds[ks - (KS - KL)][q][tid] = wt[nt][ks].p[q];
+        for (int q = 0; q < NB; ++q) w_lds[ks - (KS - KL)][q][tid] = wt[nt][ks].p[q];
       }
     }
   }
@@ -425,6 +604,8 @@
     const long long d_t0 = clock64();
 #endif
     float keep_z[NTW][4];
+    float dA[G][NTW][4];
+    unsigned amax = 0;
     float cg[G][NTW][4], ca[NTW][4], cprev[NTW][4], cd[NTW][4];
 #pragma unroll
     for (int r = 0; r < 4; ++r)
@@ -491,13 +672,40 @@
         }
 #pragma unroll
         for (int gt = 0; gt < G; ++gt) {
-          unsigned short dw[3];
-          split_scalar((KIND == 1 && gt == 2) ? dgh_n : dpre[gt], dw);
-#pragma unroll
-          for (int q = 0; q < 3; ++q) dg_pl[q][row_i][gt * H + u] = dw[q];
+          const float da = (KIND == 1 && gt == 2) ? dgh_n : dpre[gt];
+          if constexpr (MATH == MATH_BF16X6) {
+            unsigned short dw[3];
+            split_scalar(da, dw);
+#pragma unroll
+            for (int q = 0; q < 3; ++q) dg_pl[q][row_i][gt * H + u] = dw[q];
+          } else {
+            dA[gt][nt][r] = da;
+            amax = max(amax, abs_bits(da));
+          }
         }
       }
     }
+    Pow2 asc{1.f, 1.f};
+    if constexpr (MATH == MATH_F16X3) {
+      const unsigned wmax = wave_max_u32(amax);
+      if (lane == 0) wave_max[wave] = wmax;
+      __syncthreads();
+      unsigned tmax = 0;
+#pragma unroll
+      for (int w4 = 0; w4 < NW / 4; ++w4) {
+        const u32x4r m4 = *reinterpret_cast<const u32x4r*>(&wave_max[4 * w4]);
+        tmax = max(tmax, max(max(m4[0], m4[1]), max(m4[2], m4[3])));
+      }
+      asc = pow2_of(tmax);
+#pragma unroll
+      for (int r = 0; r < 4; r += 2)
+#pragma unroll
+        for (int nt = 0; nt < NTW; ++nt)
+#pragma unroll
+          for (int gt = 0; gt < G; ++gt)
+            store_pair_f16(dA[gt][nt][r] * asc.down, dA[gt][nt][r + 1] * asc.down,
+                           &dg_pl[0][quad * 4 + r][gt * H + wave * (H / NW) + nt * 16 + l15], 16 * LDGB, LDGB);
+    }
 #ifdef RNN_SEQ_DBG_TIME
     const long long d_t1 = clock64();
 #endif
@@ -505,27 +713,35 @@
 #ifdef RNN_SEQ_DBG_TIME
     const long long d_t2 = clock64();
 #endif
-    f32x4 acc[NTW];
-#pragma unroll
-    for (int nt = 0; nt < NTW; ++nt) acc[nt] = f32x4{0.f, 0.f, 0.f, 0.f};
+    f32x4 acc[NTW], lo[NTW];
+#pragma unroll
+    for (int nt = 0; nt < NTW; ++nt) {
+      acc[nt] = f32x4{0.f, 0.f, 0.f, 0.f};
+      if constexpr (MATH == MATH_F16X3) lo[nt] = acc[nt];
+    }
 #pragma unroll
     for (int ks = 0; ks < KS; ++ks) {
-      bf16x8 a[3];
-#pragma unroll
-      for (int q = 0; q < 3; ++q)
+      bf16x8 a[NA];
+#pragma unroll
+      for (int q = 0; q < NA; ++q)
         a[q] = *reinterpret_cast<const bf16x8*>(&dg_pl[q][l15][32 * ks + 8 * quad]);
-      Planes3 wl;
+      WFrag<MATH> wl;
       const bool from_lds = KL > 0 && ks >= KS - KL;
       if (from_lds) {
 #pragma unroll
-        for (int q = 0; q < 3; ++q) wl.p[q] = w_lds[KL > 0 ? ks - (KS - KL) : 0][q][tid];
-      }
-#pragma unroll
-      for (int q = 0; q < 6; ++q)
-#pragma unroll
-        for (int nt = 0; nt < NTW; ++nt) {
-          const bf16x8 wb = (from_lds && nt == 0) ? wl.p[X3_PB[q]] : wt[nt][ks].p[X3_PB[q]];
-          acc[nt] = __builtin_amdgcn_mfma_f32_16x16x32_bf16(a[X3_PA[q]], wb, acc[nt], 0, 0, 0);
+        for (int q = 0; q < NB; ++q) wl.p[q] = w_lds[KL > 0 ? ks - (KS - KL) : 0][q][tid];
+      }
+#pragma unroll
+      for (int q = 0; q < NP; ++q)
+#pragma unroll
+        for (int nt = 0; nt < NTW; ++nt)
+        {
+          if constexpr (MATH == MATH_F16X3) {
+            f16x3_mfma(q, a, wt[nt][ks], acc[nt], lo[nt]);
+          } else {
+            const bf16x8 wb = (from_lds && nt == 0) ? wl.p[X3_PB[q]] : wt[nt][ks].p[X3_PB[q]];
+            acc[nt] = __builtin_amdgcn_mfma_f32_16x16x32_bf16(a[X3_PA[q]], wb, acc[nt], 0, 0, 0);
+          }
         }
     }
 #pragma unroll
@@ -533,12 +749,17 @@
       const bool active = s < len[r];
       if (active)
 #pragma unroll
-        for (int nt = 0; nt < NTW; ++nt) dh[nt][r] = acc[nt][r] + keep_z[nt][r];
+        for (int nt = 0; nt < NTW; ++nt) {
+          if constexpr (MATH == MATH_F16X3)
+            dh[nt][r] = fmaf(lo[nt][r], F16X3_POST, acc[nt][r]) * wpost[nt] * asc.up + keep_z[nt][r];
+          else
+            dh[nt][r] = acc[nt][r] + keep_z[nt][r];
+        }
     }
 #ifdef RNN_SEQ_DBG_TIME
     const long long d_t3 = clock64();
 #endif
-    __syncthreads();
+    if constexpr (MATH == MATH_BF16X6) __syncthreads();
 #ifdef RNN_SEQ_DBG_TIME
     const long long d_t4 = clock64();
     d_a += d_t1 - d_t0;
@@ -554,27 +775,53 @@
 #endif
 }
 
-template <int KIND>
+int rnn_math(const char* who) {
+  const int m = vlnce_opt(VLNCE_OPT_RNN_MATH);
+  if (m < 1 || m > 3) {
+    vlnce_set_error("%s: option rnn_math must be 1 (bf16 planes, six products), 2 (fp16 planes, three products, on "
+                    "the instances measured faster) or 3 (fp16 planes everywhere), not %d", who, m);
+    return -1;
+  }
+  return m;
+}
+int fwd_math(int opt, int , int H) {
+  return (opt == 3 || (opt == 2 && H == 128)) ? MATH_F16X3 : MATH_BF16X6;
+}
+int bwd_math(int opt, int kind, int H) {
+  return (opt == 3 || (opt == 2 && (H == 128 || kind == 1))) ? MATH_F16X3 : MATH_BF16X6;
+}
+
+template <int KIND, int MATH>
 int launch_fwd(const RnnSeqParams& p, int H, int dirs, hipStream_t s) {
   dim3 grid(ceil_div(p.B, 16), dirs);
   if (H == 64)
-    hipLaunchKernelGGL((rnn_seq_fwd_kernel<KIND, 64, 4>), grid, dim3(256), 0, s, p);
+    hipLaunchKernelGGL((rnn_seq_fwd_kernel<KIND, 64, 4, MATH>), grid, dim3(256), 0, s, p);
   else if (H == 128)
-    hipLaunchKernelGGL((rnn_seq_fwd_kernel<KIND, 128, 8>), grid, dim3(512), 0, s, p);
+    hipLaunchKernelGGL((rnn_seq_fwd_kernel<KIND, 128, 8, MATH>), grid, dim3(512), 0, s, p);
   else
     return 1;
   return 0;
 }
-template <int KIND>
+int launch_fwd(int kind, int opt, const RnnSeqParams& p, int H, int dirs, hipStream_t s) {
+  if (fwd_math(opt, kind, H) == MATH_F16X3)
+    return kind == 0 ? launch_fwd<0, MATH_F16X3>(p, H, dirs, s) : launch_fwd<1, MATH_F16X3>(p, H, dirs, s);
+  return kind == 0 ? launch_fwd<0, MATH_BF16X6>(p, H, dirs, s) : launch_fwd<1, MATH_BF16X6>(p, H, dirs, s);
+}
+template <int KIND, int MATH>
 int launch_bwd(const RnnSeqParams& p, int H, int dirs, hipStream_t s) {
   dim3 grid(ceil_div(p.B, 16), dirs);
   if (H == 64)
-    hipLaunchKernelGGL((rnn_seq_bwd_kernel<KIND, 64, 4>), grid, dim3(256), 0, s, p);
+    hipLaunchKernelGGL((rnn_seq_bwd_kernel<KIND, 64, 4, MATH>), grid, dim3(256), 0, s, p);
   else if (H == 128)
-    hipLaunchKernelGGL((rnn_seq_bwd_kernel<KIND, 128, 8>), grid, dim3(512), 0, s, p);
+    hipLaunchKernelGGL((rnn_seq_bwd_kernel<KIND, 128, 8, MATH>), grid, dim3(512), 0, s, p);
   else
     return 1;
   return 0;
+}
+int launch_bwd(int kind, int opt, const RnnSeqParams& p, int H, int dirs, hipStream_t s) {
+  if (bwd_math(opt, kind, H) == MATH_F16X3)
+    return kind == 0 ? launch_bwd<0, MATH_F16X3>(p, H, dirs, s) : launch_bwd<1, MATH_F16X3>(p, H, dirs, s);
+  return kind == 0 ? launch_bwd<0, MATH_BF16X6>(p, H, dirs, s) : launch_bwd<1, MATH_BF16X6>(p, H, dirs, s);
 }
 
 }
@@ -587,7 +834,10 @@
                                  const float* const* w_hh, const float* const* b_hh,
                                  const int* lengths, float* const* out, float* const* h_final,
                                  float* const* gates_save, float* const* aux_save, int B, int L,
-                                 int H, vlnce_stream_t stream) {
+                                 int H, const int* options, vlnce_stream_t stream) {
+  VlnceOptScope opt_scope(options);
+  const int math = rnn_math("rnn_seq_fwd");
+  if (math < 0) return 1;
   VLNCE_CHECK_ARG(gi && w_hh && b_hh && lengths && out && h_final, "rnn_seq_fwd: null argument");
   VLNCE_CHECK_ARG(dirs == 1 || dirs == 2, "rnn_seq_fwd: dirs must be 1 or 2");
   VLNCE_CHECK_ARG(vlnce_rnn_seq_supported(kind, H), "rnn_seq_fwd: unsupported kind/H (%d,%d)", kind, H);
@@ -608,7 +858,7 @@
   p.B = B;
   p.L = L;
   hipStream_t s = reinterpret_cast<hipStream_t>(stream);
-  const int rc = kind == 0 ? launch_fwd<0>(p, H, dirs, s) : launch_fwd<1>(p, H, dirs, s);
+  const int rc = launch_fwd(kind, math, p, H, dirs, s);
   VLNCE_CHECK_ARG(rc == 0, "rnn_seq_fwd: no kernel for H=%d", H);
   VLNCE_CHECK_LAUNCH("rnn_seq_fwd");
   return 0;
@@ -619,7 +869,10 @@
                                  const float* const* gates_save, const float* const* aux_save,
                                  const float* const* dout, const float* const* dh_final,
                                  float* const* dgi, float* const* dgh, int B, int L, int H,
-                                 vlnce_stream_t stream) {
+                                 const int* options, vlnce_stream_t stream) {
+  VlnceOptScope opt_scope(options);
+  const int math = rnn_math("rnn_seq_bwd");
+  if (math < 0) return 1;
   VLNCE_CHECK_ARG(w_hh_t && lengths && out && gates_save && aux_save && dgi,
                   "rnn_seq_bwd: null argument");
   VLNCE_CHECK_ARG(dirs == 1 || dirs == 2, "rnn_seq_bwd: dirs must be 1 or 2");
@@ -640,7 +893,7 @@
   p.B = B;
   p.L = L;
   hipStream_t s = reinterpret_cast<hipStream_t>(stream);
-  const int rc = kind == 0 ? launch_bwd<0>(p, H, dirs, s) : launch_bwd<1>(p, H, dirs, s);
+  const int rc = launch_bwd(kind, math, p, H, dirs, s);
   VLNCE_CHECK_ARG(rc == 0, "rnn_seq_bwd: no kernel for H=%d", H);
   VLNCE_CHECK_LAUNCH("rnn_seq_bwd");
   return 0;
@@ -652,7 +905,10 @@
                                   const int* lengths, float* const* out_tm, float* seq,
                                   long seq_st, long seq_sb, float* const* h_final,
                                   float* const* gates_save, float* const* aux_save, int B, int L,
-                                  int H, vlnce_stream_t stream) {
+                                  int H, const int* options, vlnce_stream_t stream) {
+  VlnceOptScope opt_scope(options);
+  const int math = rnn_math("rnn_seq_fwd2");
+  if (math < 0) return 1;
   VLNCE_CHECK_ARG(gi && w_hh && b_hh && lengths && out_tm && h_final, "rnn_seq_fwd2: null argument");
   VLNCE_CHECK_ARG(dirs == 1 || dirs == 2, "rnn_seq_fwd2: dirs must be 1 or 2");
   VLNCE_CHECK_ARG(vlnce_rnn_seq_supported(kind, H), "rnn_seq_fwd2: unsupported kind/H (%d,%d)", kind, H);
@@ -678,7 +934,7 @@
   p.B = B;
   p.L = L;
   hipStream_t s = reinterpret_cast<hipStream_t>(stream);
-  const int rc = kind == 0 ? launch_fwd<0>(p, H, dirs, s) : launch_fwd<1>(p, H, dirs, s);
+  const int rc = launch_fwd(kind, math, p, H, dirs, s);
   VLNCE_CHECK_ARG(rc == 0, "rnn_seq_fwd2: no kernel for H=%d", H);
   VLNCE_CHECK_LAUNCH("rnn_seq_fwd2");
   return 0;
@@ -689,7 +945,10 @@
                                   const float* const* aux_save, const float* dseq, long dseq_st,
                                   long dseq_sb, float* dout_ws, const float* const* dh_final,
                                   float* const* dgi, float* const* dgh, int B, int L, int H,
-                                  vlnce_stream_t stream) {
+                                  const int* options, vlnce_stream_t stream) {
+  VlnceOptScope opt_scope(options);
+  const int math = rnn_math("rnn_seq_bwd2");
+  if (math < 0) return 1;
   VLNCE_CHECK_ARG(w_hh && lengths && out_tm && gates_save && aux_save && dgi,
                   "rnn_seq_bwd2: null argument");
   VLNCE_CHECK_ARG(dirs == 1 || dirs == 2, "rnn_seq_bwd2: dirs must be 1 or 2");
@@ -721,7 +980,7 @@
   p.lengths = lengths;
   p.B = B;
   p.L = L;
-  const int rc = kind == 0 ? launch_bwd<0>(p, H, dirs, s) : launch_bwd<1>(p, H, dirs, s);
+  const int rc = launch_bwd(kind, math, p, H, dirs, s);
   VLNCE_CHECK_ARG(rc == 0, "rnn_seq_bwd2: no kernel for H=%d", H);
   VLNCE_CHECK_LAUNCH("rnn_seq_bwd2");
   return 0;
diff --git a/vln-ce_amd/ops.py b/vln-ce_amd/ops.py
--- a/vln-ce_amd/ops.py
+++ b/vln-ce_amd/ops.py
@@ -1056,6 +1056,7 @@
         lib.rnn_seq_fwd2(kind, dirs, gis, w_hh, b_hh, lengths, out_tm, seq, dirs * H, Lm * dirs * H,
                          hfin, gates, aux, B, Lm, H)
         ctx.cfg = (kind, dirs, Lm, B, H, GH, E, ldx)
+        ctx.rnn_math = lib.effective_option("rnn_math") if hasattr(lib, "effective_option") else None
         ctx.set_materialize_grads(False)
         if save:
             ctx.save_for_backward(lengths, x_tm, *w_ih, *w_hh, *out_tm, *gates, *aux)
@@ -1087,7 +1088,8 @@
         lib = L()
         ws = new(dirs, Lm, B, H) if dseq is not None else None
         lib.rnn_seq_bwd2(kind, dirs, list(w_hh), lengths, list(out_tm), list(gates), list(aux), dseq,
-                         st, sb, ws, dhf, dgi, dgh, B, Lm, H)
+                         st, sb, ws, dhf, dgi, dgh, B, Lm, H,
+                         **({"options": {"rnn_math": ctx.rnn_math}} if ctx.rnn_math is not None else {}))
         dw_ih = [new(GH, E) for _ in range(dirs)]
         dw_hh = [new(GH, H) for _ in range(dirs)]
         db_ih = [new(GH) for _ in range(dirs)]
```

Result: no change. 8321 (-1.0%).
